# audexdev/Lossless-Audio-Codec

Hardware: AMD Instinct MI355X
Metric: encode Msamples/s at 1/2/4/8 MI355X; byte-identical .lac vs CPU ref (higher is better)
Workload: dtype int64

## Files before the change

### lossless-audio-codec_amd/csrc/analyze_core.h

```cpp
#pragma once
#include <type_traits>

#include "lacx_types.h"
#include "x87.h"

namespace lacx {

template <int CH_, int T_>
struct Geo {
    static constexpr int CH = CH_;
    static constexpr int T = T_;
    static constexpr int MAXN = CH_ * T_;
    static constexpr int LV = (CH_ == 16) ? 5 : ((CH_ == 8) ? 4 : 3);
    static constexpr int TPG = 64 / CH_;
    static constexpr int NG = MAXN / 64;
    static constexpr int W256 = 256 / CH_;
    static constexpr int W96 = 96 / CH_;
    static constexpr int MAXP = (MAXN >= 8192) ? 8 : ((MAXN >= 4096) ? 7 : ((MAXN >= 2048) ? 6 : ((MAXN >= 1024) ? 5 : ((MAXN >= 512) ? 4 : 3))));
    static constexpr int NSEG = (2 << MAXP) - 2;
    static_assert(32 % CH_ == 0, "chunk must divide the 96/256 windows");
    static_assert(MAXN % 64 == 0, "whole groups");
};

template <class G>
LACX_HD int sw(int j) {
    return (j % G::CH) * G::T + (j / G::CH);
}

enum : int { PCM_PLANAR_I32 = 0, PCM_INTERLEAVED_I16 = 1, PCM_INTERLEAVED_I24 = 2 };

struct SlotSrc {
    const int32_t* a;
    const int32_t* b;
    int kind;
    int layout = PCM_PLANAR_I32;
    int channels = 2;
};

LACX_HD int32_t sext24(uint32_t v) { return (int32_t)(v << 8) >> 8; }
LACX_HD int32_t slot_combine(int kind, int32_t l, int32_t r);

LACX_HD int32_t slot_fetch(const SlotSrc& s, int64_t idx) {
    int32_t l, r = 0;
    if (s.layout == PCM_PLANAR_I32) {
        if (s.kind == CH_L) return s.a[idx];
        if (s.kind == CH_R) return s.b[idx];
        l = s.a[idx];
        r = s.b[idx];
    } else if (s.layout == PCM_INTERLEAVED_I16) {
        if (s.channels == 2) {
            const uint32_t w = reinterpret_cast<const uint32_t*>(s.a)[idx];
            l = (int32_t)(int16_t)(w & 0xFFFFu);
            r = (int32_t)(int16_t)(w >> 16);
        } else {
            l = reinterpret_cast<const int16_t*>(s.a)[idx];
        }
    } else {
        const uint8_t* p = reinterpret_cast<const uint8_t*>(s.a) + idx * 3 * s.channels;
        l = sext24((uint32_t)p[0] | ((uint32_t)p[1] << 8) | ((uint32_t)p[2] << 16));
        if (s.channels == 2) r = sext24((uint32_t)p[3] | ((uint32_t)p[4] << 8) | ((uint32_t)p[5] << 16));
    }
    return slot_combine(s.kind, l, r);
}

LACX_HD uint32_t zigzag32(int32_t r) { return ((uint32_t)r << 1) ^ (uint32_t)(r >> 31); }

LACX_HD int opaque_i32(int v) {
#if defined(__HIP_DEVICE_COMPILE__)
    asm volatile("" : "+v"(v));
#endif
    return v;
}

LACX_HD int ctz32(uint32_t v) {
    return __builtin_ctz(v);
}

LACX_HD int clz32(uint32_t v) {
#if defined(__HIP_DEVICE_COMPILE__)
    return __clz((int)v);
#else
    return v ? __builtin_clz(v) : 32;
#endif
}

LACX_HD uint32_t kmean(uint64_t S, uint32_t c) {
    const uint64_t X = S + (c >> 1);
    const uint64_t Y = X - c;
    const int g = clz64((uint64_t)c) - clz64(Y);
    const uint32_t k = (uint32_t)g + ((Y >> (g & 63)) >= c ? 1u : 0u);
    return (X < 2ull * c) ? 0u : k;
}
LACX_HD uint32_t kmean32(uint32_t S, uint32_t c) {
    const uint32_t X = S + (c >> 1);
    const uint32_t Y = X - c;
    const int g = clz32(c) - clz32(Y);
    const uint32_t k = (uint32_t)g + ((Y >> (g & 31)) >= c ? 1u : 0u);
    return (X < 2u * c) ? 0u : k;
}

constexpr uint64_t kNarrowLimit = (1ull << 32) - (1ull << 20);

template <bool NARROW>
LACX_HD uint32_t kmean_t(uint64_t S, uint32_t c) {
    return NARROW ? kmean32((uint32_t)S, c) : kmean(S, c);
}

LACX_HD uint64_t rice_cost(uint32_t u, uint32_t k) {
    return (uint64_t)((k >= 31u) ? 0u : (u >> k)) + 1u + k;
}

LACX_HD uint32_t flag01(bool b) {
    uint32_t v = b ? 1u : 0u;
#if defined(__HIP_DEVICE_COMPILE__)
    asm volatile("" : "+v"(v));
#endif
    return v;
}

template <bool NARROW, bool STEADY = false>
LACX_HD uint32_t biased_k(uint32_t km, uint64_t P, uint64_t W, uint32_t d, uint32_t c) {
    const uint32_t L = NARROW ? ((((uint32_t)P - (uint32_t)W) + 128u) >> 8) : (uint32_t)(((P - W) + 128u) >> 8);
    const uint32_t U = (3u * L + 3u) >> 2;
    const uint32_t D = L + (L + 3u) / 3u + 1u;
    const uint64_t X = NARROW ? (uint64_t)((uint32_t)P + (c >> 1)) : P + (c >> 1);
    const uint64_t Uc = (uint64_t)U * c, Dc = (uint64_t)D * c;
    uint32_t act = flag01(X >= (uint64_t)c);
    if (!STEADY) act &= flag01(c > 256u);
    const int32_t drift = (int32_t)(act & flag01(X < Uc)) - (int32_t)(act & flag01(X >= Dc));
    const uint32_t large = d & 0xFFFFu, zero = d >> 16;
    uint32_t big = flag01(large >= 72u), sml = flag01(zero >= 77u);
    if (!STEADY) {
        const uint32_t m = flag01(c >= 96u);
        big &= m;
        sml &= m;
    }
    sml &= big ^ 1u;
    int32_t bias = drift + (int32_t)big - (int32_t)sml;
    bias = bias < -1 ? -1 : (bias > 1 ? 1 : bias);
    int bk = (int)km + bias;
    bk = bk < 0 ? 0 : (bk > 31 ? 31 : bk);
    return (uint32_t)bk;
}

struct SegInfo {
    uint64_t sbits;
    uint8_t ak;
    uint8_t sk;
    uint8_t pad[6];
};

template <class G>
struct PartMem {
    uint32_t grp[15][G::NG + 1];
    SegInfo seginfo[G::NSEG];
    unsigned long long segacc[G::NSEG][3];
    uint32_t segrun[G::NSEG];
    uint8_t choice[G::NSEG];
    unsigned long long pbits[G::MAXP + 1];
    uint32_t qcount;
    uint32_t wqcount[16];
    uint16_t queue[G::T * G::MAXP];
};

constexpr int kEmitTileWords = 12288;
template <class G>
struct EmitOut {
    uint32_t obits[kEmitTileWords];
    uint8_t kin[G::MAXN];
};
struct NoEmitOut {};

template <class G>
struct Smem {
    uint32_t u[G::MAXN + 4];
    union XP {
        int32_t x[G::MAXN];
        PartMem<G> part;
        typename std::conditional<G::T == 1024, EmitOut<G>, NoEmitOut>::type o;
    } xp;
    uint64_t tabP[G::T + 1];
    int32_t tabNZ[G::T + 1];
    uint32_t tabF[G::T + 1];
    uint16_t tabZM[G::T];
    uint16_t tabLM[G::T];
    uint16_t tabUZ[G::T + 2];
    uint16_t bqueue[G::T];
    uint32_t bqcount;
    uint32_t planeTot[2][32];
    uint32_t planeTot256[2][32];
    unsigned long long acc[2][4];
    uint32_t lbacc[11][3];
    uint32_t has4[2];
    uint64_t wtotP[16];
    int32_t wtotZ[16];
    uint32_t wtotF[16];
    uint64_t best_bits, best_rice, best_zr, best_bin, best_static;
    uint32_t best_k0, best_sk, best_hasrun;
    int32_t best_cand;
    int32_t next_cand;
    uint64_t cand_key[11];
    uint32_t cur_k0;
    LpcSet lpc;
    ChannelPlan plan;
    int32_t tabNX[G::T + 1];
    int32_t wx[16];
    uint8_t part_mode_k[kMaxParts];
    uint32_t ptype, order, p, parts, cand, header_bits, payload_bytes;
    uint32_t err;
    uint32_t plan_any_zr;
    uint32_t tmpl_state, tmpl_pad[3];
};

template <class G>
struct Thread {
    int tid;
    int a;
    uint32_t n;
    int cnt;
    uint32_t cs[G::LV];
    unsigned long long crice, cbin, czr;
    uint32_t chasrun;
    uint32_t has4;
    uint32_t umin;
    uint32_t zmask;
};

template <class G>
LACX_HD void thread_init(Thread<G>& th, uint32_t n, int tid) {
    th.tid = tid;
    th.a = tid * G::CH;
    th.n = n;
    const int rem = (int)n - th.a;
    th.cnt = rem < 0 ? 0 : (rem > G::CH ? G::CH : rem);
}

LACX_HD int32_t slot_combine(int kind, int32_t l, int32_t r) {
    if (kind == CH_L) return l;
    if (kind == CH_R) return r;
    if (kind == CH_M) return (int32_t)((uint32_t)l + (uint32_t)r) >> 1;
    return (int32_t)((uint32_t)l - (uint32_t)r);
}

struct alignas(16) Vec16 {
    uint32_t w[4];
};

template <int NV>
LACX_HD void load_vec16(const void* p, uint32_t* w ) {
    const Vec16* q = static_cast<const Vec16*>(p);
#pragma unroll
    for (int k = 0; k < NV; ++k) {
        const Vec16 t = q[k];
        w[4 * k] = t.w[0];
        w[4 * k + 1] = t.w[1];
        w[4 * k + 2] = t.w[2];
        w[4 * k + 3] = t.w[3];
    }
}

LACX_HD uint32_t bytes3(uint32_t lo, uint32_t hi, int sh) {
    const uint32_t x = sh == 0 ? lo : sh == 1 ? (lo >> 8) : sh == 2 ? ((lo >> 16) | (hi << 16)) : ((lo >> 24) | (hi << 8));
    return x & 0xFFFFFFu;
}

LACX_HD bool aligned16(const void* p) { return (reinterpret_cast<uintptr_t>(p) & 15u) == 0; }

template <int CH>
LACX_HD bool span_ok(const SlotSrc& s, int64_t first) {
    if (s.layout == PCM_PLANAR_I32) {
        const bool needa = s.kind != CH_R, needb = s.kind != CH_L;
        return CH % 4 == 0 && (!needa || aligned16(s.a + first)) && (!needb || aligned16(s.b + first));
    }
    const uint8_t* base = reinterpret_cast<const uint8_t*>(s.a);
    if (s.layout == PCM_INTERLEAVED_I16)
        return s.channels == 2 ? (CH % 4 == 0 && aligned16(base + first * 4)) : (CH % 8 == 0 && aligned16(base + first * 2));
    return CH % 16 == 0 && aligned16(base + first * (s.channels == 2 ? 6 : 3));
}

template <int CH>
LACX_HD void stage_span(const SlotSrc& s, int64_t first, int32_t* v) {
    if (s.layout == PCM_PLANAR_I32) {
        constexpr int NV = CH / 4 > 0 ? CH / 4 : 1;
        const bool needa = s.kind != CH_R, needb = s.kind != CH_L;
        uint32_t la[4 * NV] = {}, lb[4 * NV] = {};
        if (needa) load_vec16<NV>(s.a + first, la);
        if (needb) load_vec16<NV>(s.b + first, lb);
#pragma unroll
        for (int i = 0; i < CH; ++i) v[i] = slot_combine(s.kind, (int32_t)la[i], (int32_t)lb[i]);
        return;
    }
    if (s.layout == PCM_INTERLEAVED_I16) {
        if (s.channels == 2) {
            constexpr int NV = CH / 4 > 0 ? CH / 4 : 1;
            uint32_t w[4 * NV];
            load_vec16<NV>(reinterpret_cast<const uint8_t*>(s.a) + first * 4, w);
#pragma unroll
            for (int i = 0; i < CH; ++i)
                v[i] = slot_combine(s.kind, (int32_t)(int16_t)(w[i] & 0xFFFFu), (int32_t)(int16_t)(w[i] >> 16));
            return;
        }
        constexpr int NV = CH / 8 > 0 ? CH / 8 : 1;
        uint32_t w[4 * NV];
        load_vec16<NV>(reinterpret_cast<const uint8_t*>(s.a) + first * 2, w);
#pragma unroll
        for (int i = 0; i < CH; ++i) v[i] = (int32_t)(int16_t)((w[(i / 2) % (4 * NV)] >> (16 * (i & 1))) & 0xFFFFu);
        return;
    }
    if (s.channels == 2) {
        constexpr int ND = CH * 6 / 4 >= 4 ? CH * 6 / 4 : 4;
        uint32_t w[ND];
        load_vec16<ND / 4>(reinterpret_cast<const uint8_t*>(s.a) + first * 6, w);
#pragma unroll
        for (int i = 0; i < CH; ++i) {
            const int ol = (i * 6) % (ND * 4), orr = (i * 6 + 3) % (ND * 4);
            v[i] = slot_combine(s.kind, sext24(bytes3(w[ol / 4], w[(ol / 4 + 1 < ND) ? ol / 4 + 1 : ol / 4], ol & 3)),
                                sext24(bytes3(w[orr / 4], w[(orr / 4 + 1 < ND) ? orr / 4 + 1 : orr / 4], orr & 3)));
        }
        return;
    }
    constexpr int ND = CH * 3 / 4 >= 4 ? CH * 3 / 4 : 4;
    uint32_t w[ND];
    load_vec16<ND / 4>(reinterpret_cast<const uint8_t*>(s.a) + first * 3, w);
#pragma unroll
    for (int i = 0; i < CH; ++i) {
        const int o = (i * 3) % (ND * 4);
        v[i] = sext24(bytes3(w[o / 4], w[(o / 4 + 1 < ND) ? o / 4 + 1 : o / 4], o & 3));
    }
}

LACX_HD bool wave_all(bool pred) {
#if defined(__HIP_DEVICE_COMPILE__)
    return __all(pred) != 0;
#else
    return pred;
#endif
}

template <int CH>
LACX_HD void load_chunk(const SlotSrc& src, int64_t first, int cnt, int64_t last, int32_t* v) {
    if (wave_all(cnt == CH && span_ok<CH>(src, first))) {
        stage_span<CH>(src, first, v);
        return;
    }
#pragma unroll
    for (int i = 0; i < CH; ++i) {
        const int64_t idx = first + i;
        v[i] = slot_fetch(src, idx < last ? idx : last);
    }
}

template <class G, class M>
LACX_HD uint32_t stage_samples(const Thread<G>& th, M& sh, const SlotSrc& src, int64_t start) {
    int32_t v[G::CH];
    load_chunk<G::CH>(src, start + th.a, th.cnt, start + (int64_t)th.n - 1, v);
    int32_t* col = &sh.xp.x[th.tid];
    uint32_t any = 0;
#pragma unroll
    for (int i = 0; i < G::CH; ++i) {
        const int32_t x = (i < th.cnt) ? v[i] : 0;
        col[i * G::T] = x;
        any |= (uint32_t)x;
    }
    return any;
}

template <int W>
LACX_HD void sliced_add(const uint32_t* a, const uint32_t* b, uint32_t* out ) {
    uint32_t carry = 0;
#pragma unroll
    for (int l = 0; l < W; ++l) {
        const uint32_t x = a[l] ^ b[l];
        out[l] = x ^ carry;
        carry = (a[l] & b[l]) | (x & carry);
    }
    out[W] = carry;
}

template <class G>
LACX_HD void plane_counts(const uint32_t* u, uint32_t* cs) {
    if (G::CH == 16) {
        uint32_t l1[8][2], l2[4][3], l3[2][4], l4[5];
#pragma unroll
        for (int i = 0; i < 8; ++i) sliced_add<1>(&u[2 * i], &u[2 * i + 1], l1[i]);
#pragma unroll
        for (int i = 0; i < 4; ++i) sliced_add<2>(l1[2 * i], l1[2 * i + 1], l2[i]);
#pragma unroll
        for (int i = 0; i < 2; ++i) sliced_add<3>(l2[2 * i], l2[2 * i + 1], l3[i]);
        sliced_add<4>(l3[0], l3[1], l4);
#pragma unroll
        for (int l = 0; l < G::LV; ++l) cs[l] = l4[l];
    } else {
        uint32_t l1[2][2], l2[3];
        sliced_add<1>(&u[0], &u[1], l1[0]);
        sliced_add<1>(&u[2], &u[3], l1[1]);
        sliced_add<2>(l1[0], l1[1], l2);
#pragma unroll
        for (int l = 0; l < G::LV; ++l) cs[l] = l2[l];
    }
}

template <class G, class M>
LACX_HD void phase_r_residual(Thread<G>& th, const M& sh, int cand, uint32_t* u ) {
    int32_t xh[G::CH + 12];
#pragma unroll
    for (int i = 0; i < G::CH + 12; ++i) {
        const int d = i - 12;
        const int co = (d >= 0) ? d / G::CH : -((-d + G::CH - 1) / G::CH);
        const int el = d - co * G::CH;
        const int tt = th.tid + co;
        const int32_t* col = &sh.xp.x[tt < 0 ? 0 : tt];
        xh[i] = (tt >= 0) ? col[el * G::T] : 0;
    }
    const int32_t* x = xh + 12;
    if (cand <= 4) {
        auto fixed = [&](auto order_tag) {
            constexpr int K = decltype(order_tag)::value;
#pragma unroll
            for (int i = 0; i < G::CH; ++i) {
                const uint32_t x0 = (uint32_t)x[i], x1 = (uint32_t)x[i - 1], x2 = (uint32_t)x[i - 2],
                               x3 = (uint32_t)x[i - 3], x4 = (uint32_t)x[i - 4];
                uint32_t r = x0;
                if (K == 1) r = x0 - x1;
                if (K == 2) r = x0 - 2u * x1 + x2;
                if (K == 3) r = x0 - 3u * x1 + 3u * x2 - x3;
                if (K == 4) r = x0 - 4u * x1 + 6u * x2 - 4u * x3 + x4;
                if (K > 0 && th.a + i < K) r = x0;
                u[i] = (i < th.cnt) ? zigzag32((int32_t)r) : 0u;
            }
        };
        if (cand == 0) fixed(std::integral_constant<int, 0>{});
        else if (cand == 1) fixed(std::integral_constant<int, 1>{});
        else if (cand == 2) fixed(std::integral_constant<int, 2>{});
        else if (cand == 3) fixed(std::integral_constant<int, 3>{});
        else fixed(std::integral_constant<int, 4>{});
    } else if (cand == 5) {
#pragma unroll
        for (int i = 0; i < G::CH; ++i) {
            const int j = th.a + i;
            const int64_t pred = (3LL * (int64_t)x[i - 1] - (int64_t)x[i - 2]) >> 2;
            const int32_t r = (j >= 2) ? (int32_t)((int64_t)x[i] - pred) : x[i];
            u[i] = (i < th.cnt) ? zigzag32(r) : 0u;
        }
    } else {
        const int ci = cand - 6;
        const int ord = sh.lpc.used[ci];
        auto lpc = [&](auto taps_tag) {
            constexpr int TAPS = decltype(taps_tag)::value;
            int32_t c[TAPS + 1];
#pragma unroll
            for (int t = 1; t <= TAPS; ++t) c[t] = (t <= ord) ? (int32_t)sh.lpc.coef[ci][t] : 0;
#pragma unroll
            for (int i = 0; i < G::CH; ++i) {
                int64_t acc = 0;
#pragma unroll
                for (int t = 1; t <= TAPS; ++t) acc += (int64_t)c[t] * (int64_t)x[i - t];
                const int32_t r = (int32_t)((int64_t)x[i] - (acc >> 15));
                u[i] = (i < th.cnt) ? zigzag32(r) : 0u;
            }
        };
        if (ord <= 4) lpc(std::integral_constant<int, 4>{});
        else if (ord <= 6) lpc(std::integral_constant<int, 6>{});
        else if (ord <= 8) lpc(std::integral_constant<int, 8>{});
        else if (ord <= 10) lpc(std::integral_constant<int, 10>{});
        else lpc(std::integral_constant<int, 12>{});
    }
}

template <class G, class M>
LACX_HD void phase_r_store(Thread<G>& th, M& sh, const uint32_t* u) {
    uint64_t s = 0;
    int32_t lastnz = -1;
#pragma unroll
    for (int i = 0; i < G::CH; ++i) {
        s += u[i];
        if (u[i] != 0) lastnz = th.a + i;
        sh.u[i * G::T + th.tid] = u[i];
    }
    sh.tabP[th.tid] = s;
    sh.tabNZ[th.tid] = lastnz;
    plane_counts<G>(u, th.cs);
}

template <class G, class M>
LACX_HD void phase_r(Thread<G>& th, M& sh, int cand) {
    uint32_t u[G::CH];
    phase_r_residual(th, sh, cand, u);
    phase_r_store(th, sh, u);
}

LACX_HD uint32_t lead_m(int32_t r) {
#if defined(__HIP_DEVICE_COMPILE__)
    uint32_t f;
    asm("v_ffbh_i32 %0, %1" : "=v"(f) : "v"(r));
    return f < 32u ? f : 32u;
#else
    const uint32_t v = (uint32_t)(r ^ (r >> 31));
    return v ? (uint32_t)__builtin_clz(v) : 32u;
#endif
}

struct BoundPartials {
    uint32_t msum;
#if defined(__HIP_DEVICE_COMPILE__)
    uint32_t code;
#else
    uint32_t nz;
    uint32_t n4;
    uint32_t ends;
    uint32_t zprev;
#endif
};

LACX_HD void bound_init(BoundPartials& b) {
#if defined(__HIP_DEVICE_COMPILE__)
    b.msum = b.code = 0;
#else
    b.msum = b.nz = b.n4 = b.ends = b.zprev = 0;
#endif
}

LACX_HD void bound_add(BoundPartials& b, int32_t r) {
    b.msum += lead_m(r);
#if defined(__HIP_DEVICE_COMPILE__)
    const uint32_t v = (uint32_t)r;
    b.code = (b.code << 2) + (v < 3u ? v : 3u);
#else
    const uint32_t z = r == 0 ? 1u : 0u;
    b.nz += z;
    b.ends += (b.zprev && !z) ? 1u : 0u;
    b.zprev = z;
    b.n4 += r == 2 ? 1u : 0u;
#endif
}

template <int CH>
LACX_HD uint32_t bound_counts(const BoundPartials& b) {
    static_assert(CH <= 16, "two bits per position in one word");
#if defined(__HIP_DEVICE_COMPILE__)
    constexpr uint32_t kLow = CH == 16 ? 0x55555555u : ((1u << (2 * (CH & 15))) - 1u) & 0x55555555u;
    const uint32_t lo = b.code & kLow, hi = (b.code >> 1) & kLow;
    const uint32_t zero = ~(lo | hi) & kLow;
    const uint32_t four = hi & ~lo;
    const uint32_t ends = zero & ~(zero << 2) & ~1u;
    return (uint32_t)__builtin_popcount(zero) | ((uint32_t)__builtin_popcount(four) << 11) |
           ((uint32_t)__builtin_popcount(ends) << 22);
#else
    return b.nz | (b.n4 << 11) | (b.ends << 22);
#endif
}

template <class G, class M>
LACX_HD void pass1_window(const Thread<G>& th, const M& sh, int32_t* xh ) {
#pragma unroll
    for (int i = 0; i < G::CH + 12; ++i) {
        const int d = i - 12;
        const int co = (d >= 0) ? d / G::CH : -((-d + G::CH - 1) / G::CH);
        const int el = d - co * G::CH;
        const int tt = th.tid + co;
        const int32_t* col = &sh.xp.x[tt < 0 ? 0 : tt];
        xh[i] = (tt >= 0) ? col[el * G::T] : 0;
    }
}

template <class G, bool FULL, class M>
LACX_HD void pass1_bounds_fixed(const Thread<G>& th, const M& sh, BoundPartials* out ) {
    int32_t xh[G::CH + 12];
    pass1_window(th, sh, xh);
    const int32_t* x = xh + 12;
    const bool first = th.a == 0;
    auto live = [&](int i, int32_t r) { return FULL ? r : ((i < th.cnt) ? r : 0); };
    {
        BoundPartials b[6];
#pragma unroll
        for (int c = 0; c < 6; ++c) bound_init(b[c]);
        const uint32_t e1 = (uint32_t)x[-1] - (uint32_t)x[-2], e1b = (uint32_t)x[-2] - (uint32_t)x[-3],
                       e1c = (uint32_t)x[-3] - (uint32_t)x[-4];
        const uint32_t e2 = e1 - e1b, e2b = e1b - e1c;
        uint32_t p1 = e1, p2 = e2, p3 = e2 - e2b;
#pragma unroll
        for (int i = 0; i < G::CH; ++i) {
            const uint32_t x0 = (uint32_t)x[i];
            const uint32_t d1 = x0 - (uint32_t)x[i - 1], d2 = d1 - p1, d3 = d2 - p2, d4 = d3 - p3;
            p1 = d1;
            p2 = d2;
            p3 = d3;
            const int32_t fir = (int32_t)(x0 - (uint32_t)((3 * x[i - 1] - x[i - 2]) >> 2));
            const bool w1 = first && i < 1, w2 = first && i < 2, w3 = first && i < 3, w4 = first && i < 4;
            bound_add(b[0], live(i, (int32_t)x0));
            bound_add(b[1], live(i, (int32_t)(w1 ? x0 : d1)));
            bound_add(b[2], live(i, (int32_t)(w2 ? x0 : d2)));
            bound_add(b[3], live(i, (int32_t)(w3 ? x0 : d3)));
            bound_add(b[4], live(i, (int32_t)(w4 ? x0 : d4)));
            bound_add(b[5], live(i, w2 ? (int32_t)x0 : fir));
        }
#pragma unroll
        for (int c = 0; c < 6; ++c) out[c] = b[c];
    }
}

template <class G, bool FULL, class M>
LACX_HD void pass1_bounds_lpc(const Thread<G>& th, const M& sh, bool lpc_off, BoundPartials* out ) {
    int32_t xh[G::CH + 12];
    pass1_window(th, sh, xh);
    const int32_t* x = xh + 12;
    auto live = [&](int i, int32_t r) { return FULL ? r : ((i < th.cnt) ? r : 0); };
    for (int ci = 0; ci < 5; ++ci) {
        BoundPartials b;
        bound_init(b);
        const int ord = lpc_off ? 0 : (int)sh.lpc.used[ci];
        auto lpc = [&](auto taps_tag) {
            constexpr int TAPS = decltype(taps_tag)::value;
            int32_t c[TAPS + 1];
#pragma unroll
            for (int t = 1; t <= TAPS; ++t) c[t] = (t <= ord) ? (int32_t)sh.lpc.coef[ci][t] : 0;
#pragma unroll
            for (int i = 0; i < G::CH; ++i) {
                int64_t acc = 0;
#pragma unroll
                for (int t = 1; t <= TAPS; ++t) acc += (int64_t)c[t] * (int64_t)x[i - t];
                const int32_t r = (int32_t)((uint32_t)x[i] - (uint32_t)((uint64_t)acc >> 15));
                bound_add(b, live(i, r));
                }
        };
        if (ord == 0) {
        } else if (ord <= 4) lpc(std::integral_constant<int, 4>{});
        else if (ord <= 6) lpc(std::integral_constant<int, 6>{});
        else if (ord <= 8) lpc(std::integral_constant<int, 8>{});
        else if (ord <= 10) lpc(std::integral_constant<int, 10>{});
        else lpc(std::integral_constant<int, 12>{});
#pragma unroll
        for (int c = 0; c < 5; ++c) {
            if (c == ci) out[c] = b;
        }
    }
}

template <class G, bool FULL, class M>
LACX_HD void pass1_bounds(const Thread<G>& th, const M& sh, bool lpc_off, BoundPartials* out ) {
    pass1_bounds_fixed<G, FULL>(th, sh, out);
    pass1_bounds_lpc<G, FULL>(th, sh, lpc_off, out + 6);
}

LACX_HD void planes_to_ksums(const uint32_t* C, uint64_t* A, int kmax) {
    uint64_t acc = 0;
#pragma unroll
    for (int b = 29; b >= 0; --b) {
        acc = (acc << 1) + C[b];
        if (b <= 15) A[b] = (b <= kmax) ? acc : 0;
    }
}

LACX_HD uint32_t pick_initial_k(const uint64_t* A, uint32_t m) {
    uint32_t best_k = 0;
    uint64_t best = ~0ull;
#pragma unroll
    for (uint32_t k = 0; k <= 12; ++k) {
        const uint64_t c = A[k] + (uint64_t)m * (1u + k);
        if (c < best) {
            best = c;
            best_k = k;
        }
    }
    return best_k;
}

LACX_HD uint32_t pick_static_k(const uint64_t* A, uint32_t m, uint64_t* bits) {
    uint32_t best_k = 0;
    uint64_t best = ~0ull;
#pragma unroll
    for (uint32_t k = 0; k <= 15; ++k) {
        const uint64_t c = A[k] + (uint64_t)m * (1u + k);
        if (c < best) {
            best = c;
            best_k = k;
        }
    }
    *bits = best;
    return best_k;
}

template <class G, bool NARROW, class M>
LACX_HD void phase_a(Thread<G>& th, M& sh) {
    uint64_t P = sh.tabP[th.tid];
    uint32_t cnt = 0;
    uint32_t c = (uint32_t)th.a;
    uint32_t zm = 0;
    uint32_t mn = 0xFFFFFFFFu;
    uint32_t fzm = 0;
    uint32_t flm = 0;
    for (int i = 0; i < th.cnt; ++i) {
        const uint32_t u = sh.u[i * G::T + th.tid];
        mn = u < mn ? u : mn;
        P += u;
        ++c;
        const uint32_t km = kmean_t<NARROW>(P, c);
        const uint32_t q = u >> km;
        const uint32_t fl = q > 3u, fz = q == 0u;
        cnt += fl + (fz << 16);
        zm |= (u == 0u ? 1u : 0u) << i;
        fzm |= fz << i;
        flm |= fl << i;
    }
    sh.tabF[th.tid] = cnt;
    sh.tabZM[th.tid] = (uint16_t)fzm;
    sh.tabLM[th.tid] = (uint16_t)flm;
    if constexpr (requires { sh.tabUZ[0]; }) sh.tabUZ[th.tid] = (uint16_t)zm;
    th.umin = mn;
    th.zmask = zm;
    const uint32_t lead = (uint32_t)ctz32(~zm);
    const int32_t before = th.a - 1 - sh.tabNZ[th.tid];
    th.has4 = (th.cnt > 0 && ((zm & (zm >> 1) & (zm >> 2) & (zm >> 3)) != 0u || (uint32_t)before + lead >= 4u)) ? 1u : 0u;
}

template <class G, class M>
LACX_HD uint32_t peek_u(const M& sh, uint32_t j, uint32_t limit) {
    const uint32_t idx = (j % (uint32_t)G::CH) * (uint32_t)G::T + (j / (uint32_t)G::CH);
    const uint32_t v = sh.u[idx] & 0x3FFFFFFFu;
    return (j < limit) ? v : 1u;
}

template <class G>
LACX_HD uint32_t window_flags(const uint32_t* tabF, int t) {
    uint32_t d = 0;
#pragma unroll
    for (int k = 1; k <= G::W96; ++k) d += (t >= k) ? tabF[t - k] : 0u;
    return d;
}

struct ChunkCosts {
    unsigned long long rice, bin, zr;
    uint32_t hasrun;
};

template <class G, bool NARROW, bool ZR = true, int TRIPS = 0, bool STEADY = false>
LACX_HD ChunkCosts phase_b_span(const Smem<G>& sh, uint32_t n, int t, int i0, int i1, uint32_t k0) {
    const int a = t * G::CH;
    uint64_t P = sh.tabP[t];
    uint64_t W = (STEADY || t >= G::W256) ? sh.tabP[t - (STEADY || t >= G::W256 ? G::W256 : 0)] : 0;
    uint32_t D = window_flags<G>(sh.tabF, t);
    const uint32_t m256 = (STEADY || t >= G::W256) ? 0xFFFFFFFFu : 0u;
    const int t256 = (STEADY || t >= G::W256) ? t - G::W256 : t;
    const int t96 = (STEADY || t >= G::W96) ? t - G::W96 : t;
    const uint32_t fin = (uint32_t)sh.tabLM[t] | ((uint32_t)sh.tabZM[t] << 16);
    const uint32_t fout = (STEADY || t >= G::W96) ? ((uint32_t)sh.tabLM[t96] | ((uint32_t)sh.tabZM[t96] << 16)) : 0u;
    uint32_t c = (uint32_t)a;
    int32_t f = a - 1 - sh.tabNZ[t];
    for (int j = 0; j < i0; ++j) {
        const uint32_t u = sh.u[j * G::T + t];
        P += u;
        ++c;
        W += sh.u[j * G::T + t256] & m256;
        D += (fin >> j) & 0x00010001u;
        D -= (fout >> j) & 0x00010001u;
        f = (f + 1) & (int32_t)(0u - flag01(u == 0u));
    }
    uint32_t kin = k0;
    if (STEADY || (c > 0u && i1 > i0)) kin = biased_k<NARROW, STEADY>(kmean_t<NARROW>(P, c), P, W, D, c);
    using Acc = typename std::conditional<NARROW, uint32_t, unsigned long long>::type;
    Acc rice = 0, bin = 0, zr = 0;
    uint32_t hasrun = 0;
    const int ifirst = i0 & (G::CH - 1);
    uint32_t w0 = sh.u[ifirst * G::T + t];
    uint32_t n1 = 1, n2 = 1, n3 = 1;
    if (ZR) {
        n1 = peek_u<G>(sh, (uint32_t)(a + i0) + 1u, n);
        n2 = peek_u<G>(sh, (uint32_t)(a + i0) + 2u, n);
        n3 = peek_u<G>(sh, (uint32_t)(a + i0) + 3u, n);
    }
    uint32_t tap256 = sh.u[ifirst * G::T + t256];
    const int last = TRIPS > 0 ? i0 + TRIPS : i1;
#pragma nounroll
    for (int i = i0; i < last; ++i) {
        const uint32_t cur256 = tap256;
        const int inext = (i + 1) & (G::CH - 1);
        const uint32_t wnext = sh.u[inext * G::T + t];
        tap256 = sh.u[inext * G::T + t256];
        const uint32_t u = w0;
        const uint32_t rc = (u >> kin) + 1u + kin;
        rice += rc;
        bin += 2u + ((u <= 4u) ? (u < 1u ? u : 1u) : rc);
        if (ZR) {
            const uint32_t z = flag01(u == 0u);
            f = (f + 1) & (int32_t)(0u - z);
            const uint32_t ahead = (n1 != 0) ? 0u : ((n2 != 0) ? 1u : ((n3 != 0) ? 2u : 3u));
            const uint32_t in4 = z & flag01((uint32_t)f + ahead >= 4u);
            const uint32_t esc = 1u << ((kin + 3u) < 24u ? (kin + 3u) : 24u);
            const uint32_t plain = 2u + ((u > esc) ? 32u : rc);
            const uint32_t token = 5u + (((uint32_t)(f - 4)) >> 2);
            const uint32_t runend = in4 & flag01(n1 != 0);
            zr += (plain & (in4 - 1u)) | (token & (0u - runend));
            hasrun |= runend;
        }
        P += u;
        ++c;
        W += cur256 & m256;
        D += (fin >> i) & 0x00010001u;
        D -= (fout >> i) & 0x00010001u;
        kin = biased_k<NARROW, STEADY>(kmean_t<NARROW>(P, c), P, W, D, c);
        w0 = wnext;
        if (ZR) {
            n1 = n2;
            n2 = n3;
            n3 = peek_u<G>(sh, (uint32_t)(a + i) + 4u, n);
        }
    }
    ChunkCosts out;
    out.rice = rice;
    out.bin = bin;
    out.zr = zr;
    out.hasrun = hasrun;
    return out;
}

template <class G, bool NARROW, bool ZR = true, bool FULL = false, bool STEADY = false>
LACX_HD void phase_b(Thread<G>& th, const Smem<G>& sh, uint32_t k0) {
    const ChunkCosts cc = phase_b_span<G, NARROW, ZR, FULL ? G::CH : 0, STEADY>(sh, th.n, th.tid, 0, th.cnt, k0);
    th.crice = cc.rice;
    th.cbin = cc.bin;
    th.czr = cc.zr;
    th.chasrun = cc.hasrun;
}

template <class G>
LACX_HD void phase_b_dispatch(Thread<G>& th, const Smem<G>& sh, uint32_t k0, bool narrow, bool zr, bool full, bool steady) {
    auto go = [&](auto narrow_t, auto zr_t) {
        constexpr bool N = decltype(narrow_t)::value, Z = decltype(zr_t)::value;
        if (full) {
            if (steady) phase_b<G, N, Z, true, true>(th, sh, k0); else phase_b<G, N, Z, true, false>(th, sh, k0);
        } else {
            if (steady) phase_b<G, N, Z, false, true>(th, sh, k0); else phase_b<G, N, Z, false, false>(th, sh, k0);
        }
    };
    if (narrow) {
        if (zr) go(std::true_type{}, std::true_type{}); else go(std::true_type{}, std::false_type{});
    } else {
        if (zr) go(std::false_type{}, std::true_type{}); else go(std::false_type{}, std::false_type{});
    }
}
template <class G>
LACX_HD void phase_b_dispatch(Thread<G>& th, const Smem<G>& sh, uint32_t k0, bool narrow, bool zr, bool full) {
    phase_b_dispatch<G>(th, sh, k0, narrow, zr, full, G::T > 64 && th.tid >= 64 && 64 * G::CH >= 256);
}

#ifndef LACX_QUEUED_STEADY
#define LACX_QUEUED_STEADY 1
#endif
template <class G>
LACX_HD void phase_b_queued(Thread<G>& th, const Smem<G>& sh, int t, uint32_t k0, bool narrow, bool zr, bool full) {
    Thread<G> c;
    thread_init(c, th.n, t);
    phase_b_dispatch<G>(c, sh, k0, narrow, zr, full, LACX_QUEUED_STEADY != 0);
    th.crice += c.crice;
    th.cbin += c.cbin;
    th.czr += c.czr;
    th.chasrun |= c.chasrun;
}

LACX_HD uint32_t census_code(uint32_t u);
LACX_HD uint32_t census_shift_sum(uint32_t cen, uint32_t K);

struct RunShape {
    uint32_t nin4, tokens, hasrun, first_in4;
};
template <int CH>
LACX_HD RunShape run_shape(uint32_t E, int32_t f) {
    RunShape r{0u, 0u, 0u, 0u};
#pragma unroll
    for (int i = 0; i < CH; ++i) {
        const uint32_t z = (E >> i) & 1u;
        f = (f + 1) & (int32_t)(0u - z);
        const uint32_t after = E >> (i + 1);
        const uint32_t ahead = (after & 1u) == 0u ? 0u : ((after & 2u) == 0u ? 1u : ((after & 4u) == 0u ? 2u : 3u));
        const uint32_t in4 = z & flag01((uint32_t)f + ahead >= 4u);
        const uint32_t runend = in4 & ((after & 1u) ^ 1u);
        r.nin4 += in4;
        r.tokens += (5u + (((uint32_t)(f - 4)) >> 2)) & (0u - runend);
        r.hasrun |= runend;
        if (i == 0) r.first_in4 = in4;
    }
    return r;
}

template <class G, bool NARROW, bool ZR>
LACX_HD bool phase_b_quick(Thread<G>& th, const Smem<G>& sh) {
    if constexpr (G::T <= 64 || 64 * G::CH <= 256) {
        return false;
    } else {
        const int t = th.tid;
        if (t < 64 || th.cnt != G::CH) return false;
        using Sum = typename std::conditional<NARROW, uint32_t, uint64_t>::type;
        const Sum P0 = (Sum)sh.tabP[t], P1 = (Sum)sh.tabP[t + 1];
        const Sum W0 = (Sum)sh.tabP[t - G::W256], W1 = (Sum)sh.tabP[t - G::W256 + 1];
        const uint32_t c0 = (uint32_t)th.a, c1 = c0 + (uint32_t)G::CH;
        const uint32_t km = kmean_t<NARROW>(P0, c1);
        uint32_t ok = flag01(km == kmean_t<NARROW>(P1, c0));
        const uint32_t Llo = (uint32_t)(((P0 - W1) + 128u) >> 8), Lhi = (uint32_t)(((P1 - W0) + 128u) >> 8);
        const uint32_t Ulo = (3u * Llo + 3u) >> 2, Uhi = (3u * Lhi + 3u) >> 2;
        const uint32_t Dlo = Llo + (Llo + 3u) / 3u + 1u, Dhi = Lhi + (Lhi + 3u) / 3u + 1u;
        const uint64_t Xlo = NARROW ? (uint64_t)((uint32_t)P0 + (c0 >> 1)) : (uint64_t)P0 + (c0 >> 1);
        const uint64_t Xhi = NARROW ? (uint64_t)((uint32_t)P1 + (c1 >> 1)) : (uint64_t)P1 + (c1 >> 1);
        const uint32_t act_never = flag01(Xhi < (uint64_t)c0), act_always = flag01(Xlo >= (uint64_t)c1);
        const uint32_t up_always = flag01(Xhi < (uint64_t)Ulo * c0), up_never = flag01(Xlo >= (uint64_t)Uhi * c1);
        const uint32_t dn_always = flag01(Xlo >= (uint64_t)Dhi * c1), dn_never = flag01(Xhi < (uint64_t)Dlo * c0);
        ok &= act_never | (act_always & (up_always | up_never) & (dn_always | dn_never));
        const int32_t drift = (int32_t)((act_never ^ 1u) & up_always) - (int32_t)((act_never ^ 1u) & dn_always);
        const uint32_t d0 = window_flags<G>(sh.tabF, t), din = sh.tabF[t], dout = sh.tabF[t - G::W96];
        const int32_t l0 = (int32_t)(d0 & 0xFFFFu), z0 = (int32_t)(d0 >> 16);
        const uint32_t big_always = flag01(l0 - (int32_t)(dout & 0xFFFFu) >= 72), big_never = flag01(l0 + (int32_t)(din & 0xFFFFu) < 72);
        uint32_t sml_always, sml_never;
        {
            const uint32_t zin = sh.tabZM[t], zout = sh.tabZM[t - G::W96];
            int32_t z = z0, zmin = z0, zmax = z0;
#pragma unroll
            for (int i = 0; i + 1 < G::CH; ++i) {
                z += (int32_t)((zin >> i) & 1u) - (int32_t)((zout >> i) & 1u);
                zmin = z < zmin ? z : zmin;
                zmax = z > zmax ? z : zmax;
            }
            sml_always = flag01(zmin >= 77);
            sml_never = flag01(zmax < 77);
        }
        ok &= big_always | (big_never & (sml_always | sml_never));
        int32_t bias = drift + (int32_t)big_always - (int32_t)((big_always ^ 1u) & sml_always);
        bias = bias < -1 ? -1 : (bias > 1 ? 1 : bias);
        int bk = (int)km + bias;
        bk = bk < 0 ? 0 : (bk > 31 ? 31 : bk);
        const uint32_t k = (uint32_t)bk;
        uint32_t any = 0;
        Sum ksum = 0;
#pragma unroll
        for (int l = 0; l < G::LV; ++l) {
            any |= th.cs[l];
            ksum += (Sum)(th.cs[l] >> k) << l;
        }
        if (ZR) ok &= flag01((any >> ((k + 3u) < 24u ? (k + 3u) : 24u)) == 0u);
        if (ok == 0u) return false;
        const Sum rice = ksum + (uint32_t)G::CH * (1u + k);
        uint32_t n14 = 0, nbig = (uint32_t)G::CH, small_shifted = 0;
        if (th.umin <= 4u) {
            uint32_t cen = 0;
#pragma unroll
            for (int i = 0; i < G::CH; ++i) cen += census_code(sh.u[i * G::T + t] & 0x3FFFFFFFu);
            n14 = ((cen >> 5) & 31u) + ((cen >> 10) & 31u) + ((cen >> 15) & 31u) + ((cen >> 20) & 31u);
            nbig = (cen >> 25) & 31u;
            small_shifted = census_shift_sum(cen, k);
        }
        th.crice = rice;
        th.cbin = (Sum)(2u * (uint32_t)G::CH + n14 + nbig * (1u + k)) + (ksum - small_shifted);
        RunShape rs{0u, 0u, 0u, 0u};
        if (ZR && th.zmask != 0u)
            rs = run_shape<G::CH>(th.zmask | (((uint32_t)sh.tabUZ[t + 1] & 7u) << G::CH), th.a - 1 - sh.tabNZ[t]);
        const uint32_t nin4 = rs.nin4, tokens = rs.tokens, hasrun = rs.hasrun;
        th.czr = ksum + (Sum)(((uint32_t)G::CH - nin4) * (3u + k) + tokens);
        th.chasrun = hasrun;
        return true;
    }
}

template <class G>
LACX_HD bool phase_b_quick_dispatch(Thread<G>& th, const Smem<G>& sh, bool narrow, bool zr) {
    if (narrow) return zr ? phase_b_quick<G, true, true>(th, sh) : phase_b_quick<G, true, false>(th, sh);
    return zr ? phase_b_quick<G, false, true>(th, sh) : phase_b_quick<G, false, false>(th, sh);
}

LACX_HD uint64_t candidate_lower_bound(uint32_t g_sum, uint32_t aux_sum, uint32_t ends, uint32_t n, int zero_run) {
    const uint32_t nzero = aux_sum & 0xFFFFu, n4 = aux_sum >> 16;
    const uint64_t lb_rice = g_sum;
    const uint64_t lb_bin = (uint64_t)g_sum - n4;
    uint64_t lb = lb_rice < lb_bin ? lb_rice : lb_bin;
    if (zero_run) {
        uint64_t zeros = 0;
        if (nzero != 0) {
            const uint32_t runs = ends > 1u ? ends : 1u;
            const uint64_t shorts = 3ull * nzero, one_long = 3ull * (runs - 1u) + 4u + ((nzero - runs + 1u) >> 2);
            zeros = shorts < one_long ? shorts : one_long;
        }
        const uint64_t lb_zr = (uint64_t)g_sum - nzero + 2ull * (n - nzero) + zeros;
        if (lb_zr < lb) lb = lb_zr;
    }
    return lb;
}

LACX_HD int candidate_at(int i) { return (int)((0x405316789A2ull >> (4 * i)) & 15ull); }

LACX_HD bool candidate_pruned(uint64_t lb, int cand, uint64_t best_bits, int best_cand) {
    return best_cand >= 0 && (lb > best_bits || (lb == best_bits && cand > best_cand));
}

template <class G>
LACX_HD void score_candidate(Smem<G>& sh, int cand, uint32_t n, int zero_run, uint32_t k0,
                             const uint32_t* planeTot, const unsigned long long* acc) {
    uint64_t A[16];
    planes_to_ksums(planeTot, A, 15);
    uint64_t sbits;
    const uint32_t sk = pick_static_k(A, n, &sbits);
    const uint64_t rice = acc[0], bin = acc[1];
    const uint32_t hasrun = acc[3] != 0;
    const uint64_t zr = (zero_run && hasrun) ? acc[2] : rice;
    uint64_t a = rice < sbits ? rice : sbits;
    uint64_t b = zr < bin ? zr : bin;
    const uint64_t best = a < b ? a : b;
    if (sh.best_cand < 0 || best < sh.best_bits || (best == sh.best_bits && cand < sh.best_cand)) {
        sh.best_cand = cand;
        sh.best_bits = best;
        sh.best_rice = rice;
        sh.best_zr = zr;
        sh.best_bin = bin;
        sh.best_static = sbits;
        sh.best_k0 = k0;
        sh.best_sk = sk;
        sh.best_hasrun = hasrun;
    }
}

LACX_HD uint32_t initial_k_from_planes(const uint32_t* planes256, uint32_t n) {
    uint64_t A[16];
    planes_to_ksums(planes256, A, 12);
    return pick_initial_k(A, n < 256u ? n : 256u);
}

LACX_HD int max_partition_order(uint32_t n) {
    int mp = 0;
    for (int p = 1; p <= kMaxPartitionOrder; ++p) {
        if ((n >> p) < (uint32_t)kMinPartition) break;
        mp = p;
    }
    return mp;
}

template <class G>
LACX_HD void packed_planes(const Thread<G>& th, uint32_t* words ) {
#pragma unroll
    for (int w = 0; w < 15; ++w) {
        uint32_t v = 0;
#pragma unroll
        for (int l = 0; l < G::LV; ++l) {
            v += (((th.cs[l] >> w) & 1u) << l) + (((th.cs[l] >> (w + 15)) & 1u) << (16 + l));
        }
        words[w] = v;
    }
}

template <class G>
LACX_HD void range_ksums(const Smem<G>& sh, uint32_t s, uint32_t e, uint64_t* A) {
#pragma unroll
    for (int k = 0; k < 16; ++k) A[k] = 0;
    const uint32_t gs = (s + 63u) >> 6, ge = e >> 6;
    uint32_t e0 = e, s1 = e;
    if (gs < ge) {
        uint32_t C[30];
#pragma unroll
        for (int w = 0; w < 15; ++w) {
            const uint32_t d = sh.xp.part.grp[w][ge] - sh.xp.part.grp[w][gs];
            C[w] = d & 0xFFFFu;
            C[w + 15] = d >> 16;
        }
        planes_to_ksums(C, A, 15);
        e0 = gs << 6;
        s1 = ge << 6;
    }
    for (uint32_t j = s; j < e0; ++j) {
        const uint32_t u = sh.u[sw<G>((int)j)];
#pragma unroll
        for (int k = 0; k < 16; ++k) A[k] += u >> k;
    }
    for (uint32_t j = s1; j < e; ++j) {
        const uint32_t u = sh.u[sw<G>((int)j)];
#pragma unroll
        for (int k = 0; k < 16; ++k) A[k] += u >> k;
    }
}

LACX_HD void seg_bounds(uint32_t n, int p, uint32_t part, uint32_t* s, uint32_t* e) {
    const uint32_t base = n >> p, parts = 1u << p;
    *s = part * base;
    *e = (part + 1u == parts) ? n : (*s + base);
}

template <class G>
LACX_HD void seg_static_eval(Smem<G>& sh, uint32_t n, int p, uint32_t part) {
    uint32_t s, e;
    seg_bounds(n, p, part, &s, &e);
    const uint32_t len = e - s;
    uint64_t A[16];
    range_ksums(sh, s, e, A);
    SegInfo si;
    si.sk = (uint8_t)pick_static_k(A, len, &si.sbits);
    const uint32_t m = len < 256u ? len : 256u;
    if (m != len) range_ksums(sh, s, s + m, A);
    si.ak = (uint8_t)pick_initial_k(A, m);
    for (int i = 0; i < 6; ++i) si.pad[i] = 0;
    sh.xp.part.seginfo[(2u << (p - 1)) - 2u + part] = si;
}

template <class G, bool NARROW, bool ZR = true, class Flush>
LACX_HD void partition_pass(const Thread<G>& th, const Smem<G>& sh, int p, Flush&& flush) {
    if (th.cnt <= 0) return;
    const uint32_t n = th.n;
    const uint32_t base = n >> p, parts = 1u << p;
    uint32_t part = (uint32_t)th.a / base;
    if (part >= parts) part = parts - 1u;
    uint32_t s = part * base;
    uint32_t e = (part + 1u == parts) ? n : s + base;
    const uint32_t segbase = (2u << (p - 1)) - 2u;
    uint64_t P = sh.tabP[th.tid];
    uint64_t Pseg;
    {
        const uint32_t cs = s / G::CH;
        Pseg = sh.tabP[cs];
        for (uint32_t j = cs * G::CH; j < s; ++j) Pseg += sh.u[sw<G>((int)j)];
    }
    int32_t lastnz = sh.tabNZ[th.tid];
    if (lastnz < (int32_t)s - 1) lastnz = (int32_t)s - 1;
    int32_t f = th.a - 1 - lastnz;
    unsigned long long rice = 0, bin = 0, zr = 0;
    uint32_t hasrun = 0;
    uint32_t u = sh.u[th.tid];
    uint32_t x1 = peek_u<G>(sh, (uint32_t)th.a + 1u, n), x2 = peek_u<G>(sh, (uint32_t)th.a + 2u, n),
             x3 = peek_u<G>(sh, (uint32_t)th.a + 3u, n);
    for (int i = 0; i < th.cnt; ++i) {
        const uint32_t j = (uint32_t)(th.a + i);
        if (j == e) {
            flush(segbase + part, rice, bin, zr, hasrun);
            rice = bin = zr = 0;
            hasrun = 0;
            ++part;
            s = e;
            e = (part + 1u == parts) ? n : s + base;
            Pseg = P;
            f = 0;
        }
        const uint32_t kin = (j == s) ? (uint32_t)sh.xp.part.seginfo[segbase + part].ak
                                      : kmean_t<NARROW>(P - Pseg, j - s);
        const uint32_t rc = ((kin >= 31u) ? 0u : (u >> kin)) + 1u + kin;
        rice += rc;
        bin += (u == 0) ? 2u : ((u <= 4u) ? 3u : 2u + rc);
        if (ZR) {
            const bool z = (u == 0);
            f = z ? f + 1 : 0;
            const uint32_t n1 = (j + 1u < e) ? x1 : 1u;
            const uint32_t n2 = (j + 2u < e) ? x2 : 1u;
            const uint32_t n3 = (j + 3u < e) ? x3 : 1u;
            const int ahead = (n1 != 0) ? 0 : ((n2 != 0) ? 1 : ((n3 != 0) ? 2 : 3));
            const bool in4 = z && (f + ahead >= 4);
            if (!in4) {
                const uint32_t esc = 1u << ((kin + 3u) < 24u ? (kin + 3u) : 24u);
                zr += 2u + ((u > esc) ? 32u : rc);
            } else if (n1 != 0) {
                zr += 2u + (((uint32_t)(f - 4)) >> 2) + 3u;
                hasrun = 1;
            }
        }
        P += u;
        u = x1;
        x1 = x2;
        x2 = x3;
        x3 = peek_u<G>(sh, (uint32_t)(th.a + i) + 4u, n);
    }
    flush(segbase + part, rice, bin, zr, hasrun);
}


template <class G>
LACX_HD bool partitions_chunk_aligned(uint32_t n, int max_p) {
    return max_p > 0 && (n % ((uint32_t)G::CH << max_p)) == 0u;
}

template <class G, bool ZR = true, class Flush>
LACX_HD void partition_fused(const Thread<G>& th, const Smem<G>& sh, int max_p, Flush&& flush) {
    const bool live = th.cnt > 0;
    const uint32_t n = th.n;
    const int t = th.tid;
    const uint32_t a = (uint32_t)th.a;
    const uint32_t Pa = (uint32_t)sh.tabP[t];
    uint32_t s[G::MAXP], rem[G::MAXP], Pseg[G::MAXP], ak[G::MAXP], sidx[G::MAXP];
    uint32_t rice[G::MAXP], bin[G::MAXP], zr[G::MAXP];
    uint32_t hasrun = 0;
#pragma unroll
    for (int q = 0; q < G::MAXP; ++q) {
        const int p = q + 1;
        rice[q] = bin[q] = zr[q] = 0;
        s[q] = rem[q] = Pseg[q] = ak[q] = sidx[q] = 0;
        if (p <= max_p) {
            const uint32_t base = n >> p;
            const uint32_t part = !live ? 0u : ((n & (n - 1u)) == 0u ? a >> (31 - clz32(n) - p) : a / base);
            s[q] = part * base;
            rem[q] = s[q] + base - a;
            Pseg[q] = (uint32_t)sh.tabP[s[q] / (uint32_t)G::CH];
            sidx[q] = (2u << (p - 1)) - 2u + part;
            ak[q] = sh.xp.part.seginfo[sidx[q]].ak;
        }
    }
    uint32_t dup = 0;
    if (!ZR) {
#pragma unroll
        for (int q = 1; q < G::MAXP; ++q)
            if (q < max_p && wave_all(s[q] == s[q - 1] && ak[q] == ak[q - 1])) dup |= 1u << q;
    }
    int32_t fg = (int32_t)a - 1 - sh.tabNZ[t];
    uint32_t P = Pa;
    uint32_t u = sh.u[t];
    uint32_t x1 = peek_u<G>(sh, a + 1u, n), x2 = peek_u<G>(sh, a + 2u, n), x3 = peek_u<G>(sh, a + 3u, n);
    auto sample = [&](int i, auto first_tag) {
        constexpr bool FIRST = decltype(first_tag)::value;
        const uint32_t j = a + (uint32_t)i;
        const bool z = (u == 0);
        fg = z ? fg + 1 : 0;
        const uint32_t ahead_g = (x1 != 0) ? 0u : ((x2 != 0) ? 1u : ((x3 != 0) ? 2u : 3u));
        const uint32_t small = (u == 0) ? 2u : 3u;
        const bool is_small = u <= 4u;
#pragma unroll
        for (int q = 0; q < G::MAXP; ++q) {
            if (q < max_p && !((dup >> q) & 1u)) {
                const uint32_t cbefore = j - s[q];
                uint32_t kin = kmean32(P - Pseg[q], FIRST ? (cbefore ? cbefore : 1u) : cbefore);
                if (FIRST) kin = (cbefore == 0) ? ak[q] : kin;
                const uint32_t rc = (u >> kin) + 1u + kin;
                rice[q] += rc;
                bin[q] += is_small ? small : 2u + rc;
                if (ZR) {
                    const uint32_t left = rem[q] - 1u - (uint32_t)i;
                    const uint32_t fp = ((uint32_t)fg < cbefore + 1u) ? (uint32_t)fg : cbefore + 1u;
                    const uint32_t ahead = ahead_g < left ? ahead_g : left;
                    const bool in4 = z & (fp + ahead >= 4u);
                    const bool runend = in4 & (ahead == 0u);
                    const uint32_t esc = 1u << ((kin + 3u) < 24u ? (kin + 3u) : 24u);
                    const uint32_t plain = 2u + ((u > esc) ? 32u : rc);
                    const uint32_t token = 5u + ((fp - 4u) >> 2);
                    zr[q] += in4 ? (runend ? token : 0u) : plain;
                    hasrun |= runend ? (1u << q) : 0u;
                }
            }
        }
        P += u;
        u = x1;
        x1 = x2;
        x2 = x3;
        x3 = peek_u<G>(sh, j + 4u, n);
    };
    if (live) {
        sample(0, std::true_type{});
        for (int i = 1; i < th.cnt; ++i) sample(i, std::false_type{});
    }
#pragma unroll
    for (int q = 1; q < G::MAXP; ++q) {
        if ((dup >> q) & 1u) {
            rice[q] = rice[q - 1];
            bin[q] = bin[q - 1];
        }
    }
#pragma unroll
    for (int q = 0; q < G::MAXP; ++q) {
        if (q < max_p) flush(q, sidx[q], rice[q], bin[q], zr[q], (hasrun >> q) & 1u);
    }
}

LACX_HD uint32_t census_code(uint32_t u) { return 1u << (5u * (u < 5u ? u : 5u)); }

template <class G>
LACX_HD uint32_t small_census(const Thread<G>& th, const Smem<G>& sh, uint32_t* u_first, uint32_t* zmask) {
    uint32_t cen = 0, zm = 0;
#pragma unroll
    for (int i = 0; i < G::CH; ++i) {
        const uint32_t u = sh.u[i * G::T + th.tid];
        if (i == 0) *u_first = u;
        cen += census_code(u);
        zm |= flag01(u == 0u) << i;
    }
    *zmask = zm;
    return cen;
}

LACX_HD uint32_t census_shift_sum(uint32_t cen, uint32_t K) {
    const uint32_t n1 = (cen >> 5) & 31u, n2 = (cen >> 10) & 31u, n3 = (cen >> 15) & 31u, n4 = (cen >> 20) & 31u;
    const uint32_t s0 = n1 + 2u * n2 + 3u * n3 + 4u * n4, s1 = n2 + n3 + 2u * n4, s2 = n4;
    return K == 0u ? s0 : (K == 1u ? s1 : (K == 2u ? s2 : 0u));
}

template <class G, class Flush, class Enqueue>
LACX_HD void partition_quick(const Thread<G>& th, const Smem<G>& sh, int max_p, Flush&& flush, Enqueue&& enqueue) {
    const bool live = th.cnt > 0;
    const uint32_t n = th.n;
    const int t = th.tid;
    const uint32_t a = (uint32_t)th.a;
    const uint32_t Pa = (uint32_t)sh.tabP[t];
    const uint32_t csum = (uint32_t)sh.tabP[t + 1] - Pa;
    uint32_t u_first;
    uint32_t zmask_unused;
    const uint32_t cen = small_census(th, sh, &u_first, &zmask_unused);
    const uint32_t u_last = sh.u[(G::CH - 1) * G::T + t];
    const uint32_t code_first = census_code(u_first);
    const bool n_pow2 = (n & (n - 1u)) == 0u;
    const int log2n = 31 - clz32(n);
    for (int q = 0; q < max_p; ++q) {
        const int p = q + 1;
        const uint32_t base = n >> p;
        const uint32_t part = !live ? 0u : (n_pow2 ? a >> (log2n - p) : a / base);
        const uint32_t s = part * base;
        const uint32_t sidx = (2u << (p - 1)) - 2u + part;
        const uint32_t Sa = Pa - (uint32_t)sh.tabP[s / (uint32_t)G::CH];
        const uint32_t ca = a - s;
        const bool head = ca == 0u;
        const uint32_t klo = kmean32(head ? u_first : Sa, ca + (uint32_t)G::CH - 1u);
        const uint32_t khi = kmean32(Sa + csum - u_last, head ? 1u : ca);
        const bool ambiguous = live && klo != khi;
        enqueue((uint32_t)t | ((uint32_t)q << 12), ambiguous);
        const bool quick = live && !ambiguous;
        const uint32_t K = klo;
        uint32_t shifted = 0;
#pragma unroll
        for (int l = 0; l < G::LV; ++l) shifted += (th.cs[l] >> K) << l;
        const uint32_t k_a = (uint32_t)sh.xp.part.seginfo[sidx].ak;
        const uint32_t rc_a = (u_first >> k_a) + 1u + k_a;
        const uint32_t ncon = (uint32_t)G::CH - (head ? 1u : 0u);
        const uint32_t cen_con = cen - (head ? code_first : 0u);
        if (head) shifted -= u_first >> K;
        const uint32_t rice = shifted + ncon * (1u + K) + (head ? rc_a : 0u);
        const uint32_t n14 = ((cen_con >> 5) & 31u) + ((cen_con >> 10) & 31u) + ((cen_con >> 15) & 31u) + ((cen_con >> 20) & 31u);
        const uint32_t nbig = (cen_con >> 25) & 31u;
        const uint32_t bin_a = 2u + (u_first <= 4u ? (u_first < 1u ? u_first : 1u) : rc_a);
        const uint32_t bin = 2u * ncon + n14 + (shifted - census_shift_sum(cen_con, K)) + nbig * (1u + K) + (head ? bin_a : 0u);
        flush(q, sidx, quick ? rice : 0u, quick ? bin : 0u, 0u, 0u);
    }
}

template <class G>
struct QuickPrep {
    uint32_t Pa, u_first, cen, code_first;
    uint32_t E;
    int32_t f0;
    RunShape rs;
    uint32_t amb;
    uint32_t Kpack[(G::MAXP + 3) / 4];
};

constexpr uint32_t kQuickMaxPairs = 256;

template <class G>
LACX_HD void partition_quick_prepare(const Thread<G>& th, const Smem<G>& sh, int max_p, QuickPrep<G>& qp) {
    const bool live = th.cnt > 0;
    const uint32_t n = th.n;
    const int t = th.tid;
    const uint32_t a = (uint32_t)th.a;
    qp.Pa = (uint32_t)sh.tabP[t];
    const uint32_t csum = (uint32_t)sh.tabP[t + 1] - qp.Pa;
    uint32_t zmask;
    qp.cen = small_census(th, sh, &qp.u_first, &zmask);
    const uint32_t u_last = sh.u[(G::CH - 1) * G::T + t];
    qp.code_first = census_code(qp.u_first);
    qp.E = zmask | (flag01(peek_u<G>(sh, a + (uint32_t)G::CH, n) == 0u) << G::CH) |
           (flag01(peek_u<G>(sh, a + (uint32_t)G::CH + 1u, n) == 0u) << (G::CH + 1)) |
           (flag01(peek_u<G>(sh, a + (uint32_t)G::CH + 2u, n) == 0u) << (G::CH + 2));
    qp.f0 = (int32_t)a - 1 - sh.tabNZ[t];
    qp.rs = run_shape<G::CH>(qp.E, qp.f0);
    uint32_t any = 0;
#pragma unroll
    for (int l = 0; l < G::LV; ++l) any |= th.cs[l];
    const bool n_pow2 = (n & (n - 1u)) == 0u;
    const int log2n = 31 - clz32(n);
    qp.amb = 0;
#pragma unroll
    for (int w = 0; w < (G::MAXP + 3) / 4; ++w) qp.Kpack[w] = 0;
#pragma unroll
    for (int q = 0; q < G::MAXP; ++q) {
        if (q >= max_p) continue;
        const int p = q + 1;
        const uint32_t base = n >> p;
        const uint32_t part = !live ? 0u : (n_pow2 ? a >> (log2n - p) : a / base);
        const uint32_t s = part * base;
        const uint32_t Sa = qp.Pa - (uint32_t)sh.tabP[s / (uint32_t)G::CH];
        const uint32_t ca = a - s;
        const bool head = ca == 0u;
        const uint32_t klo = kmean32(head ? qp.u_first : Sa, ca + (uint32_t)G::CH - 1u);
        const uint32_t khi = kmean32(Sa + csum - u_last, head ? 1u : ca);
        const bool cut_front = (qp.E & 1u) != 0u && (uint32_t)qp.f0 > ca;
        const bool cut_back = ca + (uint32_t)G::CH == base && ((qp.E >> (G::CH - 1)) & 3u) == 3u;
        const bool escape = (any >> ((klo + 3u) < 24u ? (klo + 3u) : 24u)) != 0u;
        const bool ambiguous = klo != khi || (cut_front && head) || cut_back || escape;
        qp.Kpack[q >> 2] |= klo << (8 * (q & 3));
        qp.amb |= (live && ambiguous) ? (1u << q) : 0u;
    }
}

template <class G, class Flush, class Enqueue>
LACX_HD void partition_quick_costs(const Thread<G>& th, const Smem<G>& sh, int max_p, const QuickPrep<G>& qp, Flush&& flush,
                                   Enqueue&& enqueue) {
    const bool live = th.cnt > 0;
    const uint32_t n = th.n;
    const int t = th.tid;
    const uint32_t a = (uint32_t)th.a;
    const bool n_pow2 = (n & (n - 1u)) == 0u;
    const int log2n = 31 - clz32(n);
    const uint32_t open_run = (uint32_t)ctz32(~qp.E);
#pragma unroll
    for (int q = 0; q < G::MAXP; ++q) {
        if (q >= max_p) continue;
        const int p = q + 1;
        const uint32_t base = n >> p;
        const uint32_t part = !live ? 0u : (n_pow2 ? a >> (log2n - p) : a / base);
        const uint32_t sidx = (2u << (p - 1)) - 2u + part;
        const uint32_t ca = a - part * base;
        const bool head = ca == 0u;
        const bool ambiguous = ((qp.amb >> q) & 1u) != 0u;
        enqueue((uint32_t)t | ((uint32_t)q << 12), ambiguous);
        const bool quick = live && !ambiguous;
        const uint32_t K = (qp.Kpack[q >> 2] >> (8 * (q & 3))) & 0xFFu;
        uint32_t shifted = 0;
#pragma unroll
        for (int l = 0; l < G::LV; ++l) shifted += (th.cs[l] >> K) << l;
        const uint32_t k_a = (uint32_t)sh.xp.part.seginfo[sidx].ak;
        const uint32_t rc_a = (qp.u_first >> k_a) + 1u + k_a;
        const uint32_t ncon = (uint32_t)G::CH - (head ? 1u : 0u);
        const uint32_t cen_con = qp.cen - (head ? qp.code_first : 0u);
        if (head) shifted -= qp.u_first >> K;
        const uint32_t rice = shifted + ncon * (1u + K) + (head ? rc_a : 0u);
        const uint32_t n14 = ((cen_con >> 5) & 31u) + ((cen_con >> 10) & 31u) + ((cen_con >> 15) & 31u) + ((cen_con >> 20) & 31u);
        const uint32_t nbig = (cen_con >> 25) & 31u;
        const uint32_t bin_a = 2u + (qp.u_first <= 4u ? (qp.u_first < 1u ? qp.u_first : 1u) : rc_a);
        const uint32_t bin = 2u * ncon + n14 + (shifted - census_shift_sum(cen_con, K)) + nbig * (1u + K) + (head ? bin_a : 0u);
        const bool head_plain = head && qp.rs.first_in4 == 0u;
        const uint32_t esc_a = 1u << ((k_a + 3u) < 24u ? (k_a + 3u) : 24u);
        const uint32_t plain_a = 2u + (qp.u_first > esc_a ? 32u : rc_a);
        const uint32_t nplain = (uint32_t)G::CH - qp.rs.nin4 - (head_plain ? 1u : 0u);
        uint32_t tokens = qp.rs.tokens;
        if ((qp.E & 1u) != 0u && (uint32_t)qp.f0 > ca && !head && open_run <= (uint32_t)G::CH)
            tokens = tokens + ((ca + open_run - 4u) >> 2) - (((uint32_t)qp.f0 + open_run - 4u) >> 2);
        const uint32_t zr = shifted + nplain * (3u + K) + (head_plain ? plain_a : 0u) + tokens;
        flush(q, sidx, quick ? rice : 0u, quick ? bin : 0u, quick ? zr : 0u, quick ? qp.rs.hasrun : 0u);
    }
}

template <class G, bool ZR = false, class Flush>
LACX_HD void partition_slow_entry(const Smem<G>& sh, uint32_t n, uint32_t entry, Flush&& flush) {
    const uint32_t t = entry & 0xFFFu;
    const int p = (int)(entry >> 12) + 1;
    const uint32_t a = t * (uint32_t)G::CH;
    const uint32_t base = n >> p;
    const uint32_t part = (n & (n - 1u)) == 0u ? a >> (31 - clz32(n) - p) : a / base;
    const uint32_t s = part * base;
    const uint32_t sidx = (2u << (p - 1)) - 2u + part;
    uint32_t S = (uint32_t)sh.tabP[t] - (uint32_t)sh.tabP[s / (uint32_t)G::CH];
    uint32_t c = a - s;
    uint32_t k = c == 0u ? (uint32_t)sh.xp.part.seginfo[sidx].ak : kmean32(S, c ? c : 1u);
    uint32_t rice = 0, bin = 0, zr = 0, hasrun = 0;
    uint32_t u = sh.u[t];
    int32_t fg = (int32_t)a - 1 - sh.tabNZ[t];
    uint32_t x1 = 1, x2 = 1, x3 = 1;
    if (ZR) {
        x1 = peek_u<G>(sh, a + 1u, n);
        x2 = peek_u<G>(sh, a + 2u, n);
        x3 = peek_u<G>(sh, a + 3u, n);
    }
#pragma unroll
    for (int i = 0; i < G::CH; ++i) {
        const uint32_t unext = ZR ? x1 : sh.u[((i + 1) & (G::CH - 1)) * G::T + t];
        const uint32_t rc = (u >> k) + 1u + k;
        rice += rc;
        bin += 2u + (u <= 4u ? (u < 1u ? u : 1u) : rc);
        if (ZR) {
            const uint32_t z = flag01(u == 0u);
            fg = (fg + 1) & (int32_t)(0u - z);
            const uint32_t ahead_g = (x1 != 0) ? 0u : ((x2 != 0) ? 1u : ((x3 != 0) ? 2u : 3u));
            const uint32_t left = base - 1u - c;
            const uint32_t fp = ((uint32_t)fg < c + 1u) ? (uint32_t)fg : c + 1u;
            const uint32_t ahead = ahead_g < left ? ahead_g : left;
            const uint32_t in4 = z & flag01(fp + ahead >= 4u);
            const uint32_t runend = in4 & flag01(ahead == 0u);
            const uint32_t esc = 1u << ((k + 3u) < 24u ? (k + 3u) : 24u);
            const uint32_t plain = 2u + ((u > esc) ? 32u : rc);
            const uint32_t token = 5u + ((fp - 4u) >> 2);
            zr += (plain & (in4 - 1u)) | (token & (0u - runend));
            hasrun |= runend;
            x1 = x2;
            x2 = x3;
            x3 = peek_u<G>(sh, a + (uint32_t)i + 4u, n);
        }
        S += u;
        ++c;
        k = kmean32(S, c);
        u = unext;
    }
    flush(sidx, rice, bin, zr, hasrun);
}

template <class G>
LACX_HD uint64_t seg_choose(Smem<G>& sh, uint32_t idx, int zero_run) {
    PartMem<G>& pm = sh.xp.part;
    const SegInfo si = pm.seginfo[idx];
    const uint64_t normal = pm.segacc[idx][0], bin = pm.segacc[idx][1];
    const bool allow_zr = zero_run && pm.segrun[idx] != 0;
    const uint64_t zr = allow_zr ? pm.segacc[idx][2] : normal;
    uint32_t mode = 0, k = si.ak;
    uint64_t bits = normal;
    if (allow_zr && zr < bits) {
        mode = 1;
        bits = zr;
    }
    if (bin < bits) {
        mode = 2;
        bits = bin;
    }
    if (si.sbits < bits || si.sbits <= bits + bits / 20u) {
        mode = 3;
        k = si.sk;
        bits = si.sbits;
    }
    pm.choice[idx] = (uint8_t)((mode << 5) | k);
    return bits;
}

template <class G>
LACX_HD void finalize_plan(Smem<G>& sh, uint32_t n, int zero_run, int max_p, ChannelPlan* out) {
    const int cand = sh.best_cand;
    uint8_t ptype, order;
    if (cand <= 4) {
        ptype = 0;
        order = (uint8_t)cand;
    } else if (cand == 5) {
        ptype = 1;
        order = 2;
    } else {
        ptype = 2;
        order = sh.lpc.used[cand - 6];
    }
    out->valid = 1;
    out->predictor_type = ptype;
    out->order = order;
    for (int i = 0; i < 12; ++i) out->coef[i] = (cand >= 6) ? sh.lpc.coef[cand - 6][i + 1] : (int16_t)0;
    const bool allow_zr = zero_run && sh.best_hasrun;
    uint32_t mode = 0, k = sh.best_k0;
    uint64_t bits = sh.best_rice;
    if (allow_zr && sh.best_zr <= bits) {
        bits = sh.best_zr;
        mode = 1;
    }
    if (sh.best_bin < bits) {
        bits = sh.best_bin;
        mode = 2;
    }
    if (sh.best_static < bits) {
        bits = sh.best_static;
        mode = 3;
        k = sh.best_sk;
    }
    uint64_t best_total = bits + 8u + 7u;
    best_total += (8u - (best_total & 7u)) & 7u;
    int best_p = 0;
    for (int p = 1; p <= max_p; ++p) {
        uint64_t total = sh.xp.part.pbits[p] + 8u + 7ull * (1u << p);
        total += (8u - (total & 7u)) & 7u;
        const uint64_t margin = best_total / 20u;
        if (total < best_total || (total <= best_total + margin && best_p == 0)) {
            best_total = total;
            best_p = p;
        }
    }
    out->partition_order = (uint8_t)best_p;
    out->total_bits = best_total;
    out->payload_bytes = (uint32_t)((16u + (ptype == 2 ? 16u * order : 0u) + best_total) >> 3);
    uint32_t any_zr = 0;
    if (best_p == 0) {
        out->part_mode_k[0] = (uint8_t)((mode << 5) | k);
        any_zr = mode == 1u;
    } else {
        const uint32_t parts = 1u << best_p, segbase = (2u << (best_p - 1)) - 2u;
        for (uint32_t i = 0; i < parts; ++i) {
            const uint8_t c = sh.xp.part.choice[segbase + i];
            out->part_mode_k[i] = c;
            any_zr |= (uint32_t)((c >> 5) == 1u);
        }
    }
    sh.plan_any_zr = any_zr;
}

}
```

### lossless-audio-codec_amd/csrc/device_util.h

```cpp
#pragma once
#include <hip/hip_runtime.h>

#include "analyze_core.h"
#include "kernels.h"

namespace lacx {

#ifdef LACX_STAMPS
extern __device__ unsigned long long g_stamp_acc[40];
#define STAMP(k)                                                        \
    do {                                                                \
        const unsigned long long _now = __builtin_amdgcn_s_memtime();   \
        stamp_acc[k] += _now - stamp_prev;                              \
        stamp_prev = _now;                                              \
    } while (0)
#define STAMP_PARAMS , unsigned long long* stamp_acc, unsigned long long& stamp_prev
#define STAMP_ARGS , stamp_acc, stamp_prev
#else
#define STAMP(k) do { } while (0)
#define STAMP_PARAMS
#define STAMP_ARGS
#endif
constexpr int kDppRowShr1 = 0x111, kDppRowShr2 = 0x112, kDppRowShr4 = 0x114, kDppRowShr8 = 0x118;
constexpr int kDppRowBcast15 = 0x142, kDppRowBcast31 = 0x143;

template <int CTRL, int ROW_MASK>
__device__ __forceinline__ uint32_t dpp_mov(uint32_t identity, uint32_t v) {
    return (uint32_t)__builtin_amdgcn_update_dpp((int)identity, (int)v, CTRL, ROW_MASK, 0xF, false);
}
template <int CTRL, int ROW_MASK>
__device__ __forceinline__ uint64_t dpp_mov64(uint64_t v) {
    const uint32_t lo = dpp_mov<CTRL, ROW_MASK>(0u, (uint32_t)v);
    const uint32_t hi = dpp_mov<CTRL, ROW_MASK>(0u, (uint32_t)(v >> 32));
    return ((uint64_t)hi << 32) | lo;
}

__device__ __forceinline__ uint32_t wave_scan_add_u32(uint32_t v) {
    v += dpp_mov<kDppRowShr1, 0xF>(0u, v);
    v += dpp_mov<kDppRowShr2, 0xF>(0u, v);
    v += dpp_mov<kDppRowShr4, 0xF>(0u, v);
    v += dpp_mov<kDppRowShr8, 0xF>(0u, v);
    v += dpp_mov<kDppRowBcast15, 0xA>(0u, v);
    v += dpp_mov<kDppRowBcast31, 0xC>(0u, v);
    return v;
}
__device__ __forceinline__ uint64_t wave_scan_add_u64(uint64_t v) {
    v += dpp_mov64<kDppRowShr1, 0xF>(v);
    v += dpp_mov64<kDppRowShr2, 0xF>(v);
    v += dpp_mov64<kDppRowShr4, 0xF>(v);
    v += dpp_mov64<kDppRowShr8, 0xF>(v);
    v += dpp_mov64<kDppRowBcast15, 0xA>(v);
    v += dpp_mov64<kDppRowBcast31, 0xC>(v);
    return v;
}
__device__ __forceinline__ int32_t wave_scan_max_i32(int32_t v) {
    constexpr uint32_t kMin = 0x80000000u;
    auto mx = [](int32_t a, uint32_t b) { return a > (int32_t)b ? a : (int32_t)b; };
    v = mx(v, dpp_mov<kDppRowShr1, 0xF>(kMin, (uint32_t)v));
    v = mx(v, dpp_mov<kDppRowShr2, 0xF>(kMin, (uint32_t)v));
    v = mx(v, dpp_mov<kDppRowShr4, 0xF>(kMin, (uint32_t)v));
    v = mx(v, dpp_mov<kDppRowShr8, 0xF>(kMin, (uint32_t)v));
    v = mx(v, dpp_mov<kDppRowBcast15, 0xA>(kMin, (uint32_t)v));
    v = mx(v, dpp_mov<kDppRowBcast31, 0xC>(kMin, (uint32_t)v));
    return v;
}
__device__ __forceinline__ uint32_t wave_scan_or_u32(uint32_t v) {
    v |= dpp_mov<kDppRowShr1, 0xF>(0u, v);
    v |= dpp_mov<kDppRowShr2, 0xF>(0u, v);
    v |= dpp_mov<kDppRowShr4, 0xF>(0u, v);
    v |= dpp_mov<kDppRowShr8, 0xF>(0u, v);
    v |= dpp_mov<kDppRowBcast15, 0xA>(0u, v);
    v |= dpp_mov<kDppRowBcast31, 0xC>(0u, v);
    return v;
}
__device__ __forceinline__ uint64_t wave_scan_min_u64(uint64_t v) {
    auto step = [](uint64_t a, uint32_t lo, uint32_t hi) {
        const uint64_t b = ((uint64_t)hi << 32) | lo;
        return b < a ? b : a;
    };
#define LACX_MIN_STEP(CTRL, MASK) \
    v = step(v, dpp_mov<CTRL, MASK>(0xFFFFFFFFu, (uint32_t)v), dpp_mov<CTRL, MASK>(0xFFFFFFFFu, (uint32_t)(v >> 32)))
    LACX_MIN_STEP(kDppRowShr1, 0xF);
    LACX_MIN_STEP(kDppRowShr2, 0xF);
    LACX_MIN_STEP(kDppRowShr4, 0xF);
    LACX_MIN_STEP(kDppRowShr8, 0xF);
    LACX_MIN_STEP(kDppRowBcast15, 0xA);
    LACX_MIN_STEP(kDppRowBcast31, 0xC);
#undef LACX_MIN_STEP
    return v;
}
__device__ __forceinline__ uint32_t wave_last_u32(uint32_t v) { return (uint32_t)__builtin_amdgcn_readlane((int)v, 63); }
__device__ __forceinline__ uint64_t wave_last_u64(uint64_t v) {
    return ((uint64_t)wave_last_u32((uint32_t)(v >> 32)) << 32) | wave_last_u32((uint32_t)v);
}
__device__ __forceinline__ uint64_t wave_sum_u64(uint64_t v) { return wave_last_u64(wave_scan_add_u64(v)); }
__device__ __forceinline__ uint32_t wave_sum_u32(uint32_t v) { return wave_last_u32(wave_scan_add_u32(v)); }
__device__ __forceinline__ uint32_t wave_or_u32(uint32_t v) { return wave_last_u32(wave_scan_or_u32(v)); }

template <int LOG>
__device__ __forceinline__ uint32_t seg_sum_u32(uint32_t v) {
    if (LOG >= 1) v += dpp_mov<kDppRowShr1, 0xF>(0u, v);
    if (LOG >= 2) v += dpp_mov<kDppRowShr2, 0xF>(0u, v);
    if (LOG >= 3) v += dpp_mov<kDppRowShr4, 0xF>(0u, v);
    if (LOG >= 4) v += dpp_mov<kDppRowShr8, 0xF>(0u, v);
    if (LOG >= 5) v += dpp_mov<kDppRowBcast15, 0xA>(0u, v);
    if (LOG >= 6) v += dpp_mov<kDppRowBcast31, 0xC>(0u, v);
    return v;
}
__device__ __forceinline__ uint32_t seg_sum_u32(uint32_t v, int log2_lanes) {
    switch (log2_lanes) {
        case 1: return seg_sum_u32<1>(v);
        case 2: return seg_sum_u32<2>(v);
        case 3: return seg_sum_u32<3>(v);
        case 4: return seg_sum_u32<4>(v);
        case 5: return seg_sum_u32<5>(v);
        default: return seg_sum_u32<6>(v);
    }
}

template <class G>
struct ScanRegs {
    uint64_t v, inc;
    int32_t z, zinc;
};

template <class G, class M>
__device__ __forceinline__ void scan_pz_part1(M& sh, int tid, ScanRegs<G>& r) {
    const int lane = tid & 63, wave = tid >> 6;
    r.v = sh.tabP[tid];
    r.z = sh.tabNZ[tid];
    const uint64_t inc = wave_scan_add_u64(r.v);
    const int32_t zinc = wave_scan_max_i32(r.z);
    r.inc = inc;
    r.zinc = zinc;
    if (lane == 63) {
        sh.wtotP[wave] = inc;
        sh.wtotZ[wave] = zinc;
    }
}

template <class G, class M>
__device__ __forceinline__ uint64_t scan_pz_part2(M& sh, int tid, const ScanRegs<G>& r) {
    const int lane = tid & 63, wave = tid >> 6;
    uint64_t base = 0, total = 0;
    int32_t zbase = -1;
#pragma unroll
    for (int w = 0; w < G::T / 64; ++w) {
        const uint64_t pw = sh.wtotP[w];
        const int32_t z = sh.wtotZ[w];
        total += pw;
        if (w < wave) {
            base += pw;
            zbase = z > zbase ? z : zbase;
        }
    }
    int32_t zprev = __shfl_up(r.zinc, 1, 64);
    if (lane == 0) zprev = -1;
    sh.tabP[tid] = base + r.inc - r.v;
    sh.tabNZ[tid] = zprev > zbase ? zprev : zbase;
    if (tid == G::T - 1) {
        sh.tabP[G::T] = base + r.inc;
        sh.tabNZ[G::T] = r.zinc > zbase ? r.zinc : zbase;
    }
    return total;
}

template <class G>
__device__ __forceinline__ void plane_totals_wave(const Thread<G>& th, uint32_t* planeTot, uint32_t* planeTot256,
                                                  int tid, int first_plane = 0) {
    const int lane = tid & 63, wave = tid >> 6;
    uint32_t any = 0;
#pragma unroll
    for (int l = 0; l < G::LV; ++l) any |= th.cs[l];
    const int nplanes = 32 - __clz((int)wave_or_u32(any));
    const uint64_t m256 = (G::W256 >= 64) ? ~0ull : ((1ull << (G::W256 & 63)) - 1ull);
    uint32_t mine = 0, mine256 = 0;
    const bool first256 = wave == 0;
    for (int b = first256 ? 0 : first_plane; b < nplanes; ++b) {
        uint32_t tot = 0, tot256 = 0;
#pragma unroll
        for (int l = 0; l < G::LV; ++l) {
            const uint64_t m = __ballot((th.cs[l] >> b) & 1u);
            tot += (uint32_t)__popcll(m) << l;
            if (first256) tot256 += (uint32_t)__popcll(m & m256) << l;
        }
        if (lane == b) {
            mine = tot;
            mine256 = tot256;
        }
    }
    if (lane < nplanes) {
        if (lane >= first_plane) atomicAdd(&planeTot[lane], mine);
        if (wave == 0) atomicAdd(&planeTot256[lane], mine256);
    }
}

template <class G>
__device__ __forceinline__ void ksums_wave(const Thread<G>& th, uint32_t* ksum, uint32_t* ksum256, int tid, uint32_t kmask = 0xFFFFu) {
    const int lane = tid & 63, wave = tid >> 6;
    static_assert(G::W256 == 16 || G::W256 == 64, "the first 256 samples are one DPP row or the whole wave");
#pragma unroll
    for (int k = 0; k < 16; ++k) {
        const bool wanted = ((kmask >> k) & 1u) != 0u;
        const bool head256 = wave == 0 && k <= 12;
        if (!wanted && !head256) continue;
        uint32_t v = 0;
#pragma unroll
        for (int l = 0; l < G::LV; ++l) v += (th.cs[l] >> k) << l;
        v += dpp_mov<kDppRowShr1, 0xF>(0u, v);
        v += dpp_mov<kDppRowShr2, 0xF>(0u, v);
        v += dpp_mov<kDppRowShr4, 0xF>(0u, v);
        v += dpp_mov<kDppRowShr8, 0xF>(0u, v);
        const uint32_t row = v;
        if (wanted || G::W256 == 64) {
            v += dpp_mov<kDppRowBcast15, 0xA>(0u, v);
            v += dpp_mov<kDppRowBcast31, 0xC>(0u, v);
            if (lane == 63) {
                if (wanted) atomicAdd(&ksum[k], v);
                if (G::W256 == 64 && wave == 0 && k <= 12) atomicAdd(&ksum256[k], v);
            }
        }
        if (G::W256 == 16 && wave == 0 && lane == 15 && k <= 12) atomicAdd(&ksum256[k], row);
    }
}

__device__ __forceinline__ uint32_t static_k_candidates(uint64_t S, uint32_t n, int lane) {
    const uint32_t k = (uint32_t)lane & 15u;
    const uint64_t fixed = (uint64_t)n * (1u + k);
    const uint64_t upper = (S >> k) + fixed;
    const uint64_t slack = (uint64_t)n * ((1u << k) - 1u);
    const uint64_t lower = (S > slack ? ((S - slack + ((1u << k) - 1u)) >> k) : 0ull) + fixed;
    const uint64_t umin = wave_last_u64(wave_scan_min_u64(lane < 16 ? upper : ~0ull));
    return (uint32_t)__ballot(lane < 16 && lower <= umin) & 0xFFFFu;
}

__device__ __forceinline__ void wave_exclusive_scan_u32(uint32_t* arr, int len, int lane) {
    uint32_t carry = 0;
    for (int base = 0; base < len; base += 64) {
        const int i = base + lane;
        const uint32_t v = (i < len) ? arr[i] : 0u;
        const uint32_t inc = wave_scan_add_u32(v);
        if (i < len) arr[i] = carry + inc - v;
        carry += wave_last_u32(inc);
    }
}

struct SlotGeom {
    int64_t start;
    uint32_t n;
    bool defined;
};

__device__ __forceinline__ uint32_t block_frames(const AnalyzeParams& prm, uint32_t blk) {
    const uint64_t rem = prm.frames - (uint64_t)blk * kMaxBlock;
    return rem < (uint64_t)kMaxBlock ? (uint32_t)rem : (uint32_t)kMaxBlock;
}

__device__ __forceinline__ SlotGeom slot_geom(const AnalyzeParams& prm, uint32_t blk, int slot) {
    SlotGeom g;
    const uint32_t nb = block_frames(prm, blk);
    const int64_t bstart = (int64_t)blk * kMaxBlock;
    const int win = slot >> 2, ch = slot & 3;
    g.defined = true;
    if (prm.channels == 1 && ch != 0) g.defined = false;
    if (win == 0) {
        g.start = bstart;
        g.n = nb;
    } else {
        if (prm.channels != 2 || prm.stereo_mode != 2 || nb <= (uint32_t)kFullCompareLimit) g.defined = false;
        g.n = kProbe;
        g.start = bstart;
        if (g.defined) {
            if (win == 2) g.start = bstart + (nb - kProbe) / 2u;
            if (win == 3) g.start = bstart + nb - kProbe;
        }
    }
    return g;
}

__device__ __forceinline__ StreamDesc wave_uniform(const StreamDesc& d) {
    static_assert(sizeof(StreamDesc) % 4 == 0, "whole words");
    StreamDesc r;
    const uint32_t* src = reinterpret_cast<const uint32_t*>(&d);
    uint32_t* dst = reinterpret_cast<uint32_t*>(&r);
#pragma unroll
    for (size_t i = 0; i < sizeof(StreamDesc) / 4; ++i) dst[i] = (uint32_t)__builtin_amdgcn_readfirstlane((int)src[i]);
    return r;
}

__device__ __forceinline__ StreamDesc stream_of_block(const BatchRef& br, uint32_t gblk) {
    if (br.table == nullptr) return br.single;
    uint32_t lo = 0, hi = br.nstreams;
    while (hi - lo > 1u) {
        const uint32_t mid = (lo + hi) >> 1;
        if (br.table[mid].first_block <= gblk) lo = mid; else hi = mid;
    }
    return br.table[lo];
}
__device__ __forceinline__ StreamDesc stream_of_block_uniform(const BatchRef& br, uint32_t gblk) {
    if (br.table == nullptr) return br.single;
    return wave_uniform(stream_of_block(br, gblk));
}
__device__ __forceinline__ StreamDesc stream_of_workgroup(const BatchRef& br, uint32_t wg) {
    if (br.table == nullptr) return br.single;
    uint32_t lo = 0, hi = br.nstreams;
    while (hi - lo > 1u) {
        const uint32_t mid = (lo + hi) >> 1;
        if (br.table[mid].first_wg <= wg) lo = mid; else hi = mid;
    }
    return wave_uniform(br.table[lo]);
}

__device__ __forceinline__ StreamDesc stream_of_item(const BatchRef& br, uint32_t item) {
    if (br.table == nullptr) return br.single;
    uint32_t lo = 0, hi = br.nstreams;
    while (hi - lo > 1u) {
        const uint32_t mid = (lo + hi) >> 1;
        if (br.table[mid].prm.stream_base <= item) lo = mid; else hi = mid;
    }
    return wave_uniform(br.table[lo]);
}

__device__ __forceinline__ SlotSrc slot_src(const AnalyzeParams& prm, const int32_t* L, const int32_t* R, int ch) {
    SlotSrc s;
    s.kind = ch;
    s.a = L;
    s.b = R;
    s.layout = prm.layout;
    s.channels = prm.channels;
    return s;
}


__device__ __forceinline__ void xcd_slot(uint32_t w, uint32_t per, uint32_t nblocks, uint32_t& blk, uint32_t& which) {
    const uint32_t group = 8u * per, g = w / group, r = w % group;
    if (g < nblocks / 8u) {
        blk = g * 8u + (r & 7u);
        which = r >> 3;
    } else {
        blk = w / per;
        which = w % per;
    }
}

constexpr unsigned long long kRecValid = 1ull << 62, kRecMs = 1ull << 61, kRecFlag = 1ull << 60, kRecBytesMask = (1ull << 60) - 1ull;

__device__ __forceinline__ unsigned long long rec_load(const unsigned long long* p) {
    return __hip_atomic_load(p, __ATOMIC_RELAXED, __HIP_MEMORY_SCOPE_AGENT);
}
__device__ __forceinline__ void rec_store(unsigned long long* p, unsigned long long v) {
    __hip_atomic_store(p, v, __ATOMIC_RELAXED, __HIP_MEMORY_SCOPE_AGENT);
}


__device__ __forceinline__ void lds_barrier() {
    asm volatile("s_waitcnt lgkmcnt(0)\n\ts_barrier" ::: "memory");
}

}
```

### lossless-audio-codec_amd/csrc/k_analyze.hip

```cpp
#include <hip/hip_runtime.h>

#include <cstdlib>
#include <mutex>

#include "emit_device.h"
#include "kernels_internal.h"

namespace lacx {

#ifdef LACX_STAMPS
__device__ unsigned long long g_stamp_acc[40];
#endif

#ifdef LACX_TEST_HOOKS
#define LACX_HOOK(prm, bits) (((prm).debug_skip & (bits)) != 0u)
#else
#define LACX_HOOK(prm, bits) false
#endif

struct PendingSlot {
    long long idx;
    uint32_t done, silent;
};

template <class G>
__device__ __forceinline__ void fused_emit(Smem<G>& sh, Thread<G>& th, const AnalyzeParams& prm, const FuseArgs& fa,
                                           const long long idx, const bool flag_byte, const uint32_t flag_value,
                                           const int tid, PendingSlot* defer, const uint32_t tmpl_key,
                                           const uint32_t* plan_stored, const int plan_words STAMP_PARAMS) {
    const uint32_t n = th.n;
    asm volatile("" : "+v"(th.tid), "+v"(th.a));
    const unsigned long long my_size = (unsigned long long)sh.plan.payload_bytes + (flag_byte ? 1u : 0u);
    if (tid == 0) rec_store(&fa.size_rec[idx], kRecValid | (flag_value ? kRecMs : 0ull) | (flag_byte ? kRecFlag : 0ull) | my_size);
    const bool skip = (unsigned long long)sh.plan.payload_bytes + 16u > fa.slot_stride ||
                      (LACX_HOOK(prm, 1024u) && (idx % 5 == 3));
    bool done = false;
    if (!skip) {
        emit_load_plan(sh, sh.plan, tid, G::T);
        __syncthreads();
        if (sh.plan_any_zr) {
            emit_first_nonzero(th, sh);
            const int32_t nxinc = scan_nx_part1<G>(sh, tid, sh.wx);
            __syncthreads();
            scan_nx_part2<G>(sh, tid, nxinc, sh.wx, (int32_t)n);
            __syncthreads();
        }
        uint8_t* slot = fa.slots + (unsigned long long)idx * fa.slot_stride;
        STAMP(24);
        done = emit_body<G>(sh, th, n, slot, fa.err_flag, [slot](uint8_t** o) { *o = slot; return true; }, tid,
                            LACX_HOOK(prm, 2048u), (uint32_t)fa.slot_stride STAMP_ARGS);
    }
    if (tmpl_key != 0u && done && sh.payload_bytes <= kSilentBytes) {
        SilentTemplate* t = fa.silent;
        if (tid == 0) sh.tmpl_state = atomicCAS(&t->state, 0u, 1u);
        __syncthreads();
        if (sh.tmpl_state == 0u) {
            const uint32_t nv = (sh.payload_bytes + 15u) >> 4;
            const uint32_t* tw = sh.xp.o.obits;
            for (uint32_t v = tid; v < nv; v += G::T) {
                uint4 o;
                o.x = __builtin_bswap32(tw[4u * v]);
                o.y = __builtin_bswap32(tw[4u * v + 1u]);
                o.z = __builtin_bswap32(tw[4u * v + 2u]);
                o.w = __builtin_bswap32(tw[4u * v + 3u]);
                reinterpret_cast<uint4*>(t->bytes)[v] = o;
            }
            if (tid < plan_words) t->plan[tid] = plan_stored[tid];
            if (tid == 0) {
                t->nbytes = sh.payload_bytes;
                t->plan_words = (uint32_t)plan_words;
            }
            asm volatile("s_waitcnt vmcnt(0)" ::: "memory");
            __syncthreads();
            if (tid == 0) __hip_atomic_store(&t->state, tmpl_key, __ATOMIC_RELEASE, __HIP_MEMORY_SCOPE_AGENT);
        }
    }
    if (defer) {
        if (tid == 0) {
            defer->idx = idx;
            defer->done = done ? 1u : 0u;
            defer->silent = LACX_HOOK(prm, 8192u) ? 1u : 0u;
        }
        return;
    }
    asm volatile("s_waitcnt vmcnt(0)" ::: "memory");
    __syncthreads();
    if (tid == 0) {
        if (done) fa.emitted[idx] = 2u;
        if (!LACX_HOOK(prm, 8192u)) rec_store(&fa.ready_rec[idx], done ? 1ull : 2ull);
    }
}

__device__ __forceinline__ void publish_pending(const FuseArgs& fa, PendingSlot& pend, int tid) {
    if (tid == 0) {
        const long long idx = pend.idx;
        if (idx >= 0) {
            if (pend.done) fa.emitted[idx] = 2u;
            if (!pend.silent) rec_store(&fa.ready_rec[idx], pend.done ? 1ull : 2ull);
        }
        pend.idx = -1;
    }
}

template <class G>
__device__ __forceinline__ void score_candidate_wave(Smem<G>& sh, int cand, uint32_t n, int zero_run, uint32_t k0,
                                                     const uint32_t* planeTot, const unsigned long long* acc, int lane,
                                                     bool ksums, uint32_t kmask) {
    uint64_t key = ~0ull;
    if (ksums) {
        if (lane < 16 && ((kmask >> lane) & 1u)) key = (((uint64_t)planeTot[lane] + (uint64_t)n * (uint64_t)(1 + lane)) << 4) | (uint64_t)lane;
    } else {
        const int b = 29 - lane;
        const uint64_t w = (lane < 30) ? ((uint64_t)planeTot[b] << b) : 0ull;
        const uint64_t tk = wave_scan_add_u64(w);
        if (lane >= 14 && lane < 30 && ((kmask >> b) & 1u)) key = (((tk >> b) + (uint64_t)n * (uint64_t)(1 + b)) << 4) | (uint64_t)b;
    }
    const uint64_t best_key = wave_last_u64(wave_scan_min_u64(key));
    if (lane == 0) {
        const uint64_t sbits = best_key >> 4;
        const uint32_t sk = (uint32_t)(best_key & 15u);
        const uint64_t rice = acc[0], bin = acc[1];
        const uint32_t hasrun = acc[3] != 0;
        const uint64_t zr = (zero_run && hasrun) ? acc[2] : rice;
        const uint64_t a = rice < sbits ? rice : sbits;
        const uint64_t c = zr < bin ? zr : bin;
        const uint64_t best = a < c ? a : c;
        if (sh.best_cand < 0 || best < sh.best_bits || (best == sh.best_bits && cand < sh.best_cand)) {
            sh.best_cand = cand;
            sh.best_bits = best;
            sh.best_rice = rice;
            sh.best_zr = zr;
            sh.best_bin = bin;
            sh.best_static = sbits;
            sh.best_k0 = k0;
            sh.best_sk = sk;
            sh.best_hasrun = hasrun;
        }
    }
}

__device__ __forceinline__ uint32_t initial_k_wave(const uint32_t* planes256, uint32_t n, int lane, bool ksums) {
    const uint32_t m = n < 256u ? n : 256u;
    uint64_t key = ~0ull;
    if (ksums) {
        if (lane <= 12) key = (((uint64_t)planes256[lane] + (uint64_t)m * (uint64_t)(1 + lane)) << 4) | (uint64_t)lane;
    } else {
        const int b = 29 - lane;
        const uint64_t w = (lane < 30) ? ((uint64_t)planes256[b] << b) : 0ull;
        const uint64_t tk = wave_scan_add_u64(w);
        if (lane >= 17 && lane < 30) key = (((tk >> b) + (uint64_t)m * (uint64_t)(1 + b)) << 4) | (uint64_t)b;
    }
    return (uint32_t)(wave_last_u64(wave_scan_min_u64(key)) & 15u);
}

template <class G>
__device__ __forceinline__ void slot_sync() {
    if constexpr (G::T == 64) {
        asm volatile("s_waitcnt lgkmcnt(0)" ::: "memory");
    } else {
        __syncthreads();
    }
}

template <class G>
__device__ __forceinline__ void analyze_slot(unsigned char* smem_raw, const AnalyzeParams& prm, uint32_t n_in,
                                             const SlotSrc& src, int64_t start, const LpcSet* __restrict__ lpc_slot,
                                             ChannelPlan* __restrict__ plan_out, int tid, const FuseArgs& fuse,
                                             const long long fuse_idx, const bool fuse_flag_byte,
                                             const uint32_t fuse_flag_value, PendingSlot* pend) {
    Smem<G>& sh = *reinterpret_cast<Smem<G>*>(smem_raw);
    const uint32_t n = n_in;
#ifdef LACX_STAMPS
    unsigned long long stamp_acc[40];
    for (int k = 0; k < 40; ++k) stamp_acc[k] = 0;
    unsigned long long stamp_prev = __builtin_amdgcn_s_memtime();
    const unsigned long long stamp_rt0 = __builtin_amdgcn_s_memrealtime();
#endif
    Thread<G> th;
    thread_init(th, n, tid);
    const uint32_t chunk_bits = stage_samples(th, sh, src, start);
    {
        const bool wave_silent = __ballot(chunk_bits != 0u) == 0ull;
        if ((tid & 63) == 0) sh.wtotF[tid >> 6] = wave_silent ? 0u : 1u;
    }
    for (int i = tid; i < (int)(sizeof(LpcSet) / 2); i += G::T)
        reinterpret_cast<uint16_t*>(&sh.lpc)[i] = reinterpret_cast<const uint16_t*>(lpc_slot)[i];
    if (tid < 32) {
        sh.planeTot[0][tid] = sh.planeTot[1][tid] = 0;
        sh.planeTot256[0][tid] = sh.planeTot256[1][tid] = 0;
    }
    if (tid < 4) sh.acc[0][tid] = sh.acc[1][tid] = 0;
    if (tid < 33) (&sh.lbacc[0][0])[tid] = 0;
    if (tid < 2) sh.has4[tid] = 0;
    if (tid == 0) {
        sh.best_cand = -1;
        sh.tabUZ[G::T] = sh.tabUZ[G::T + 1] = 0;
    }
    if (pend) asm volatile("s_waitcnt vmcnt(0)" ::: "memory");
    slot_sync<G>();
    if (pend) publish_pending(fuse, *pend, tid);
    STAMP(0);

    auto run_pass1 = [&](const bool real) {
        asm volatile("" : "+v"(th.a));
        const bool lpc_off = LACX_HOOK(prm, 16u);
        const uint32_t per_thread = 34u * (uint32_t)G::CH;
        const int32_t left = (int32_t)n - (int32_t)((tid >> 6) * 64 * G::CH);
        const uint32_t valid = left <= 0 ? 0u : (left >= 64 * G::CH ? (uint32_t)(64 * G::CH) : (uint32_t)left);
        const uint32_t beyond = (uint32_t)(64 * G::CH) - valid;
        auto reduce_pair = [&](int c0, const BoundPartials& b0, bool two, const BoundPartials& b1) {
            const uint32_t lo = per_thread - b0.msum, hi = two ? per_thread - b1.msum : 0u;
            const uint32_t g2 = wave_sum_u32(lo | (hi << 16));
            const uint32_t cnt0 = wave_sum_u32(bound_counts<G::CH>(b0));
            const uint32_t cnt1 = two ? wave_sum_u32(bound_counts<G::CH>(b1)) : 0u;
            if ((tid & 63) == 0 && real) {
#pragma unroll
                for (int h = 0; h < 2; ++h) {
                    if (h == 0 || two) {
                        const uint32_t g = h ? (g2 >> 16) : (g2 & 0xFFFFu);
                        const uint32_t cnt = h ? cnt1 : cnt0;
                        const uint32_t nz = cnt & 0x7FFu, n4 = (cnt >> 11) & 0x7FFu, ends = cnt >> 22;
                        atomicAdd(&sh.lbacc[c0 + h][0], g - nz - beyond);
                        atomicAdd(&sh.lbacc[c0 + h][1], (nz - beyond) + (n4 << 16));
                        atomicAdd(&sh.lbacc[c0 + h][2], ends);
                    }
                }
            }
        };
        {
            BoundPartials bf[6];
            if (n == (uint32_t)G::MAXN) pass1_bounds_fixed<G, true>(th, sh, bf);
            else pass1_bounds_fixed<G, false>(th, sh, bf);
#pragma unroll
            for (int c = 0; c < 6; c += 2) reduce_pair(c, bf[c], true, bf[c + 1]);
        }
        asm volatile("" : "+v"(th.a));
        {
            BoundPartials bl[5];
            if (n == (uint32_t)G::MAXN) pass1_bounds_lpc<G, true>(th, sh, lpc_off, bl);
            else pass1_bounds_lpc<G, false>(th, sh, lpc_off, bl);
            reduce_pair(6, bl[0], true, bl[1]);
            reduce_pair(8, bl[2], true, bl[3]);
            reduce_pair(10, bl[4], false, bl[4]);
        }
    };
    bool silent = true;
#pragma unroll
    for (int w = 0; w < G::T / 64; ++w) silent = silent && sh.wtotF[w] == 0u;
    uint32_t tmpl_key = 0;
    if (silent) {
        uint32_t key = 0;
        if constexpr (G::T == 1024) {
            if (fuse.silent && !LACX_HOOK(prm, ~0u)) {
                key = 0x80000000u | (prm.zero_run ? 0x40000000u : 0u) | (prm.partitioning ? 0x20000000u : 0u) | n;
                if (tid == 0) sh.tmpl_state = __hip_atomic_load(&fuse.silent->state, __ATOMIC_RELAXED, __HIP_MEMORY_SCOPE_AGENT);
            }
        }
        STAMP(2);
        slot_sync<G>();
        if constexpr (G::T == 1024) {
            if (key) {
                const uint32_t state = (uint32_t)__builtin_amdgcn_readfirstlane((int)sh.tmpl_state);
                if (state == key) {
                    __builtin_amdgcn_fence(__ATOMIC_ACQUIRE, "agent");
                    const SilentTemplate* t = fuse.silent;
                    const uint32_t nbytes = t->nbytes;
                    if (tid == 0 && fuse.silent_copies) atomicAdd(fuse.silent_copies, 1u);
                    if ((uint32_t)tid < t->plan_words) reinterpret_cast<uint32_t*>(plan_out)[tid] = t->plan[tid];
                    if (fuse_idx >= 0) {
                        if (tid == 0)
                            rec_store(&fuse.size_rec[fuse_idx], kRecValid | (fuse_flag_value ? kRecMs : 0ull) | (fuse_flag_byte ? kRecFlag : 0ull) |
                                                                    ((unsigned long long)nbytes + (fuse_flag_byte ? 1u : 0u)));
                        typedef unsigned int u32x4 __attribute__((ext_vector_type(4)));
                        uint8_t* slot = fuse.slots + (unsigned long long)fuse_idx * fuse.slot_stride;
                        const __amdgpu_buffer_rsrc_t rsrc = __builtin_amdgcn_make_buffer_rsrc(slot, 0, (int)fuse.slot_stride, 0x00020000);
                        const uint32_t nv = (nbytes + 15u) >> 4;
                        for (uint32_t v = tid; v < nv; v += G::T) {
                            const uint4 w = reinterpret_cast<const uint4*>(t->bytes)[v];
                            u32x4 o;
                            o.x = w.x;
                            o.y = w.y;
                            o.z = w.z;
                            o.w = w.w;
                            __builtin_amdgcn_raw_buffer_store_b128(o, rsrc, (int)(16u * v), 0, 16 );
                        }
                        if (pend) {
                            if (tid == 0) {
                                pend->idx = fuse_idx;
                                pend->done = 1u;
                                pend->silent = 0u;
                            }
                        } else {
                            asm volatile("s_waitcnt vmcnt(0)" ::: "memory");
                            __syncthreads();
                            if (tid == 0) {
                                fuse.emitted[fuse_idx] = 2u;
                                rec_store(&fuse.ready_rec[fuse_idx], 1ull);
                            }
                        }
                    }
                    return;
                }
                if (state == 0u && fuse_idx >= 0) tmpl_key = key;
            }
        }
        if (tid <= 10) sh.cand_key[tid] = tid == 0 ? 0ull : ~0ull;
    } else {
#if defined(LACX_STAMPS) && LACX_STAMPS == 3
    {
        uint32_t trips = 2;
        asm volatile("" : "+s"(trips));
        for (uint32_t r = 0; r < trips; ++r) {
            run_pass1(r == 0);
            if (r == 0) STAMP(2); else STAMP(15);
        }
    }
#else
    run_pass1(true);
    STAMP(2);
#endif
    slot_sync<G>();
    if (tid <= 10) {
        const bool avail = !((tid >= 6 && (sh.lpc.used[tid >= 6 ? tid - 6 : 0] == 0 || LACX_HOOK(prm, 16u))) ||
                             (tid >= 1 && LACX_HOOK(prm, 64u)));
        sh.cand_key[tid] = avail ? ((candidate_lower_bound(sh.lbacc[tid][0], sh.lbacc[tid][1], sh.lbacc[tid][2], n, prm.zero_run) << 4) | (uint64_t)tid)
                                 : ~0ull;
    }
    }
    STAMP(5);

    int pending = -1;
    uint32_t pending_k0 = 0;
    bool pending_ksums = false;
    uint32_t pending_kmask = 0xFFFFu;
    uint32_t tried = 0;
    int parity = 0;
    for (;;) {
        asm volatile("" : "+v"(tid));
        if (tid < 64) {
            if (pending >= 0) {
                score_candidate_wave(sh, pending, n, prm.zero_run, pending_k0, sh.planeTot[parity ^ 1], sh.acc[parity ^ 1], tid, pending_ksums, pending_kmask);
                if (tid < 32) sh.planeTot[parity ^ 1][tid] = sh.planeTot256[parity ^ 1][tid] = 0;
                if (tid < 4) sh.acc[parity ^ 1][tid] = 0;
            }
            const uint64_t key = (tid <= 10 && !((tried >> tid) & 1u)) ? sh.cand_key[tid] : ~0ull;
            const uint64_t best_key = wave_last_u64(wave_scan_min_u64(key));
            if (tid == 0) {
                sh.has4[parity] = 0;
                sh.bqcount = 0;
                int next = best_key == ~0ull ? -1 : (int)(best_key & 15u);
                if (next >= 0 && !LACX_HOOK(prm, 128u) && candidate_pruned(best_key >> 4, next, sh.best_bits, sh.best_cand)) next = -1;
                sh.next_cand = next;
            }
        }
        STAMP(1);
        slot_sync<G>();
        STAMP(4);
        const int cand = sh.next_cand;
        if (cand < 0) break;
        tried |= 1u << cand;
        asm volatile("" : "+v"(th.a));
        uint32_t* pt = sh.planeTot[parity];
        uint32_t* pt256 = sh.planeTot256[parity];
        unsigned long long* acc = sh.acc[parity];
        {
            uint32_t ures[G::CH];
            phase_r_residual(th, sh, cand, ures);
            phase_r_store(th, sh, ures);
        }
        ScanRegs<G> sr;
        scan_pz_part1(sh, tid, sr);
        STAMP(3);
        slot_sync<G>();
        const uint64_t total_u = scan_pz_part2(sh, tid, sr);
        const bool narrow = total_u < kNarrowLimit;
        const bool ksums = narrow && !LACX_HOOK(prm, 262144u);
        const uint32_t kmask = !LACX_HOOK(prm, 1048576u) ? static_k_candidates(total_u, n, tid & 63) : 0xFFFFu;
        if (!LACX_HOOK(prm, 1u)) {
            if (ksums) ksums_wave(th, pt, pt256, tid, kmask);
            else plane_totals_wave(th, pt, pt256, tid, kmask ? (int)__builtin_ctz(kmask) : 0);
        }
        if (tid < 64) {
            const uint32_t k0w = initial_k_wave(pt256, n, tid, ksums);
            if (tid == 0) sh.cur_k0 = k0w;
        }
        STAMP(6);
        if (LACX_HOOK(prm, 2u)) {
            sh.tabF[tid] = 0;
            th.has4 = 1u;
        } else if (narrow) {
            phase_a<G, true>(th, sh);
        } else {
            phase_a<G, false>(th, sh);
        }
        if (__ballot(th.has4 != 0u) != 0ull && (tid & 63) == 0) sh.has4[parity] = 1u;
        STAMP(8);
        slot_sync<G>();
        STAMP(10);
        const uint32_t k0 = sh.cur_k0;
        asm volatile("" : "+v"(th.tid));
        if (LACX_HOOK(prm, 4u)) {
            th.crice = th.cbin = th.czr = 1;
            th.chasrun = 0;
        } else {
            const bool zr = prm.zero_run && sh.has4[parity] != 0u;
            const bool full = n == (uint32_t)G::MAXN;
            if (G::T == 64 || LACX_HOOK(prm, 524288u)) {
                phase_b_dispatch<G>(th, sh, k0, narrow, zr, full);
                if ((uint32_t)th.a >= n) {
                    th.crice = th.cbin = th.czr = 0;
                    th.chasrun = 0;
                }
            } else {
                const bool live = (uint32_t)th.a < n;
                bool quick = false;
                if (tid >= 64 && live) quick = phase_b_quick_dispatch<G>(th, sh, narrow, zr);
                if (!quick) {
                    th.crice = th.cbin = th.czr = 0;
                    th.chasrun = 0;
                }
                if (tid >= 64) {
                    const unsigned long long slow = __ballot(live && !quick);
                    if (slow != 0ull) {
                        uint32_t base = 0;
                        if ((tid & 63) == 0) base = atomicAdd(&sh.bqcount, (uint32_t)__popcll(slow));
                        base = (uint32_t)__builtin_amdgcn_readfirstlane((int)base);
                        if (live && !quick) sh.bqueue[base + __builtin_amdgcn_mbcnt_hi((uint32_t)(slow >> 32), __builtin_amdgcn_mbcnt_lo((uint32_t)slow, 0u))] = (uint16_t)tid;
                    }
                }
                STAMP(11);
                slot_sync<G>();
                if (tid < 64) {
                    if (live) phase_b_dispatch<G>(th, sh, k0, narrow, zr, full, false);
                } else {
                    const int w = tid >> 6;
                    const int order = (w & 3) ? (w - 1 - (w >> 2)) : (11 + (w >> 2));
                    const uint32_t qn = sh.bqcount;
                    for (uint32_t e0 = (uint32_t)order * 64u; e0 < qn; e0 += 15u * 64u) {
                        const uint32_t e = e0 + (uint32_t)(tid & 63);
                        if (e < qn) phase_b_queued<G>(th, sh, (int)sh.bqueue[e], k0, narrow, zr, full);
                    }
                }
            }
        }
        STAMP(12);
        {
            const uint64_t r0 = wave_sum_u64(th.crice);
            const uint64_t r1 = wave_sum_u64(th.cbin);
            const uint64_t r2 = wave_sum_u64(th.czr);
            const uint32_t r3 = wave_or_u32(th.chasrun);
            if ((tid & 63) == 0) {
                atomicAdd(&acc[0], (unsigned long long)r0);
                atomicAdd(&acc[1], (unsigned long long)r1);
                atomicAdd(&acc[2], (unsigned long long)r2);
                atomicAdd(&acc[3], (unsigned long long)r3);
            }
        }
        STAMP(13);
        slot_sync<G>();
        STAMP(14);
        pending = cand;
        pending_k0 = k0;
        pending_ksums = ksums;
        pending_kmask = kmask;
        parity ^= 1;
    }

    STAMP(15);
    asm volatile("" : "+v"(tid), "+v"(th.tid), "+v"(th.a));
    const int best = sh.best_cand;
    int max_p = 0;
    if (prm.partitioning && n >= (uint32_t)kMinPartition) max_p = max_partition_order(n);
    const int nseg = max_p > 0 ? ((2 << max_p) - 2) : 0;
    PartMem<G>& pm = sh.xp.part;
    auto clear_partition_scratch = [&]() {
        for (int i = tid; i < nseg; i += G::T) {
            pm.segacc[i][0] = pm.segacc[i][1] = pm.segacc[i][2] = 0;
            pm.segrun[i] = 0;
        }
        if (tid <= G::MAXP) pm.pbits[tid] = 0;
    };
    if (best == pending && !LACX_HOOK(prm, 16384u)) {
        clear_partition_scratch();
        slot_sync<G>();
    } else {
        phase_r(th, sh, best);
        ScanRegs<G> sr;
        scan_pz_part1(sh, tid, sr);
        slot_sync<G>();
        clear_partition_scratch();
        scan_pz_part2(sh, tid, sr);
        slot_sync<G>();
    }
    const bool pnarrow = sh.tabP[G::T] < kNarrowLimit;
    STAMP(16);
    if (max_p > 0) {
        {
            constexpr int kLog = G::TPG == 4 ? 2 : 4;
            static_assert(G::TPG == 4 || G::TPG == 16, "lanes per 64-sample group");
            uint32_t words[15];
            packed_planes(th, words);
            const bool last = (tid & (G::TPG - 1)) == G::TPG - 1;
#pragma unroll
            for (int w = 0; w < 15; ++w) {
                const uint32_t v = seg_sum_u32<kLog>(words[w]);
                if (last) pm.grp[w][tid / G::TPG] = v;
            }
            if (tid < 15) pm.grp[tid][G::NG] = 0;
        }
        slot_sync<G>();
        {
            constexpr int NW = G::T / 64;
            const int wave = tid >> 6, lane = tid & 63;
            for (int w = wave; w < 15; w += NW) wave_exclusive_scan_u32(pm.grp[w], G::NG + 1, lane);
        }
        slot_sync<G>();
        STAMP(17);
        for (int idx = tid; idx < (LACX_HOOK(prm, 32u) ? 0 : nseg); idx += G::T) {
            const int p = 31 - __clz(idx + 2);
            seg_static_eval(sh, n, p, (uint32_t)(idx + 2 - (1 << p)));
        }
        slot_sync<G>();
        STAMP(18);
        auto flush = [&pm](uint32_t idx, unsigned long long rc, unsigned long long bn, unsigned long long zr,
                           uint32_t hr) {
            atomicAdd(&pm.segacc[idx][0], rc);
            atomicAdd(&pm.segacc[idx][1], bn);
            atomicAdd(&pm.segacc[idx][2], zr);
            if (hr) atomicOr(&pm.segrun[idx], 1u);
        };
        if (LACX_HOOK(prm, 8u)) {
        } else if (pnarrow && partitions_chunk_aligned<G>(n, max_p)) {
            const bool ablate_flush = LACX_HOOK(prm, 65536u);
            const uint32_t chunks = n / (uint32_t)G::CH;
            const bool pow2 = (chunks & (chunks - 1u)) == 0u && !LACX_HOOK(prm, 131072u);
            auto seg_flush = [&](int q, uint32_t idx, uint32_t rc, uint32_t bn, uint32_t zr, uint32_t hr, bool with_zr) {
                if (ablate_flush) return;
                const uint32_t lanes = chunks >> (q + 1);
                if (pow2 && lanes >= 2u) {
                    const int lg = lanes >= 64u ? 6 : 31 - __clz((int)lanes);
                    const bool last = ((uint32_t)tid & ((1u << lg) - 1u)) == (1u << lg) - 1u;
                    rc = seg_sum_u32(rc, lg);
                    bn = seg_sum_u32(bn, lg);
                    if (with_zr) zr = seg_sum_u32(zr, lg);
                    if (last) {
                        atomicAdd(reinterpret_cast<uint32_t*>(&pm.segacc[idx][0]), rc);
                        atomicAdd(reinterpret_cast<uint32_t*>(&pm.segacc[idx][1]), bn);
                        if (with_zr) atomicAdd(reinterpret_cast<uint32_t*>(&pm.segacc[idx][2]), zr);
                    }
                } else {
                    atomicAdd(reinterpret_cast<uint32_t*>(&pm.segacc[idx][0]), rc);
                    atomicAdd(reinterpret_cast<uint32_t*>(&pm.segacc[idx][1]), bn);
                    if (with_zr) atomicAdd(reinterpret_cast<uint32_t*>(&pm.segacc[idx][2]), zr);
                }
                if (hr) atomicOr(&pm.segrun[idx], 1u);
            };
            auto flush32 = [&](int q, uint32_t idx, uint32_t rc, uint32_t bn, uint32_t zr, uint32_t hr) {
                seg_flush(q, idx, rc, bn, zr, hr, true);
            };
            auto flush32_nozr = [&](int q, uint32_t idx, uint32_t rc, uint32_t bn, uint32_t, uint32_t) {
                seg_flush(q, idx, rc, bn, 0u, 0u, false);
            };
            auto flush_entry = [&pm, ablate_flush](uint32_t idx, uint32_t rc, uint32_t bn, uint32_t zr, uint32_t hr) {
                if (ablate_flush) return;
                atomicAdd(reinterpret_cast<uint32_t*>(&pm.segacc[idx][0]), rc);
                atomicAdd(reinterpret_cast<uint32_t*>(&pm.segacc[idx][1]), bn);
                if (zr) atomicAdd(reinterpret_cast<uint32_t*>(&pm.segacc[idx][2]), zr);
                if (hr) atomicOr(&pm.segrun[idx], 1u);
            };
            const bool with_zr = prm.zero_run && sh.best_hasrun;
            if (LACX_HOOK(prm, 32768u)) {
                if (with_zr) partition_fused<G, true>(th, sh, max_p, flush32);
                else partition_fused<G, false>(th, sh, max_p, flush32_nozr);
            } else {
                uint16_t* wq = &pm.queue[(tid >> 6) * 64 * G::MAXP];
                uint32_t queued = 0;
                auto enqueue = [&](uint32_t entry, bool ambiguous) {
                    const unsigned long long m = __ballot(ambiguous);
                    if (ambiguous) wq[queued + __builtin_amdgcn_mbcnt_hi((uint32_t)(m >> 32), __builtin_amdgcn_mbcnt_lo((uint32_t)m, 0u))] = (uint16_t)entry;
                    queued += (uint32_t)__popcll(m);
                };
                asm volatile("" : "+v"(th.tid));
                if (!with_zr) {
                    partition_quick<G>(th, sh, max_p, flush32_nozr, enqueue);
                } else {
                    QuickPrep<G> qp;
                    partition_quick_prepare<G>(th, sh, max_p, qp);
                    uint32_t pairs = 0;
                    for (int q = 0; q < max_p; ++q) pairs += (uint32_t)__popcll(__ballot((qp.amb >> q) & 1u));
                    if (pairs > kQuickMaxPairs) partition_fused<G, true>(th, sh, max_p, flush32);
                    else partition_quick_costs<G>(th, sh, max_p, qp, flush32, enqueue);
                }
                STAMP(7);
                if constexpr (G::T > 64) {
                    constexpr int NW = G::T / 64;
                    static_assert(NW <= 16, "one count per wave");
                    const int lane = tid & 63;
                    if (lane == 0) pm.wqcount[tid >> 6] = queued;
                    __syncthreads();
                    const uint32_t mine = lane < NW ? pm.wqcount[lane] : 0u;
                    const uint32_t incl = wave_scan_add_u32(mine);
                    const uint32_t total = (uint32_t)__builtin_amdgcn_readlane((int)incl, NW - 1);
                    for (uint32_t e0 = (uint32_t)(tid & ~63); e0 < total; e0 += (uint32_t)G::T) {
                        const bool live = e0 + (uint32_t)lane < total;
                        const uint32_t e = live ? e0 + (uint32_t)lane : total - 1u;
                        uint32_t w = 0;
#pragma unroll
                        for (int step = NW / 2; step >= 1; step >>= 1) {
                            const uint32_t probe = (uint32_t)__shfl((int)incl, (int)(w + (uint32_t)step - 1u), 64);
                            w += probe <= e ? (uint32_t)step : 0u;
                        }
                        const uint32_t prev = (uint32_t)__shfl((int)incl, (int)(w ? w - 1u : 0u), 64);
                        const uint32_t before = w ? prev : 0u;
                        const uint32_t entry = pm.queue[w * 64u * (uint32_t)G::MAXP + (e - before)];
                        if (live) {
                            if (with_zr) partition_slow_entry<G, true>(sh, n, entry, flush_entry);
                            else partition_slow_entry<G, false>(sh, n, entry, flush_entry);
                        }
                    }
                } else {
                    asm volatile("s_waitcnt lgkmcnt(0)" ::: "memory");
                    for (uint32_t e = (uint32_t)(tid & 63); e < queued; e += 64u) {
                        if (with_zr) partition_slow_entry<G, true>(sh, n, wq[e], flush_entry);
                        else partition_slow_entry<G, false>(sh, n, wq[e], flush_entry);
                    }
                }
                STAMP(9);
            }
        } else {
            for (int p = 1; p <= max_p; ++p) {
                if (pnarrow) {
                    partition_pass<G, true>(th, sh, p, flush);
                } else {
                    partition_pass<G, false>(th, sh, p, flush);
                }
            }
        }
        STAMP(19);
        slot_sync<G>();
        STAMP(20);
        for (int j0 = tid & ~63; j0 < nseg + 2; j0 += G::T) {
            const int j = j0 + (tid & 63), idx = j - 2;
            const bool valid = j >= 2 && idx < nseg;
            const unsigned long long bits = valid ? seg_choose(sh, (uint32_t)idx, prm.zero_run) : 0ull;
            if (j0 >= 64) {
                const unsigned long long sum = wave_sum_u64(bits);
                if ((tid & 63) == 0) atomicAdd(&pm.pbits[31 - __clz(j0)], sum);
            } else if (valid) {
                atomicAdd(&pm.pbits[31 - __clz(j)], bits);
            }
        }
        slot_sync<G>();
    }
    if (tid == 0) finalize_plan(sh, n, prm.zero_run, max_p, &sh.plan);
    slot_sync<G>();
    const int plan_words = (int)(offsetof(ChannelPlan, part_mode_k) + ((size_t)1 << sh.plan.partition_order) + 3) / 4;
    for (int i = tid; i < plan_words; i += G::T)
        reinterpret_cast<uint32_t*>(plan_out)[i] = reinterpret_cast<const uint32_t*>(&sh.plan)[i];
    STAMP(21);
    if constexpr (G::T == 1024) {
        if (fuse_idx >= 0) fused_emit<G>(sh, th, prm, fuse, fuse_idx, fuse_flag_byte, fuse_flag_value, tid, pend, tmpl_key,
                                        reinterpret_cast<const uint32_t*>(plan_out), plan_words STAMP_ARGS);
    }
    STAMP(23);
#if defined(LACX_STAMPS) && (LACX_STAMPS == 1 || LACX_STAMPS == 3)
    if ((tid & 63) == 0 && (tid >> 6) == (int)(blockIdx.x & 15u) && G::T == 1024) {
        stamp_acc[22] = __builtin_amdgcn_s_memrealtime() - stamp_rt0;
        for (int k = 0; k < 32; ++k) atomicAdd(&g_stamp_acc[k], stamp_acc[k]);
        atomicAdd(&g_stamp_acc[32], 1ull);
    }
#endif
}

#ifndef LACX_PROBE_WAVES
#define LACX_PROBE_WAVES 6
#endif
#ifndef LACX_PROBE_WG_WAVES
#define LACX_PROBE_WG_WAVES 1
#endif
constexpr int kProbeWaves = LACX_PROBE_WG_WAVES;
template <class G>
struct TailArgs {};
template <>
struct TailArgs<GProbe> {
    uint32_t* front_ctr;
    BlockPlan* bplans;
    uint32_t* need_full_out;
};
template <class G>
__global__ __launch_bounds__(G::T == 64 ? 64 * kProbeWaves : G::T, G::T == 64 ? LACX_PROBE_WAVES : 4) void k_analyze(BatchRef br, int probe_class, uint32_t one_block,
                                                  int which_base, const LpcSet* __restrict__ lpcs,
                                                  const uint32_t* __restrict__ need,
                                                  ChannelPlan* __restrict__ plans,
                                                  unsigned long long* __restrict__ t_first,
                                                  unsigned long long* __restrict__ t_last, FuseArgs fuse,
                                                  uint32_t* __restrict__ work_ctr, uint32_t total_wg, uint32_t pair_blocks,
                                                  TailArgs<G> tail) {
    extern __shared__ __align__(16) unsigned char smem_all[];
    __shared__ uint32_t s_next;
    __shared__ PendingSlot s_pend;
    static_assert(sizeof(Smem<G>) % 16 == 0, "slot images are 16-byte aligned");
    const int tid = G::T == 64 ? (int)(threadIdx.x & 63u) : (int)threadIdx.x;
    unsigned char* smem_raw = smem_all + (G::T == 64 ? (size_t)(threadIdx.x >> 6) * sizeof(Smem<G>) : 0);
    if (t_first && tid == 0) atomicMax(t_first, ~(unsigned long long)__builtin_amdgcn_s_memrealtime());
    const bool persistent = work_ctr != nullptr;
    uint32_t rep = 0;
    uint32_t v = G::T == 64 ? blockIdx.x * (uint32_t)kProbeWaves + (uint32_t)__builtin_amdgcn_readfirstlane((int)(threadIdx.x >> 6)) : blockIdx.x;
    if (persistent) {
        if (tid == 0) {
            s_next = atomicAdd(work_ctr, 1u);
            s_pend.idx = -1;
        }
        __syncthreads();
        v = (uint32_t)__builtin_amdgcn_readfirstlane((int)s_next);
    }
    for (;;) {
        if (persistent && v >= total_wg) break;
        uint32_t blk;
        uint32_t reps = 1u;
        int slot = -1;
        int which_in_block = -1;
        uint32_t needed_slots = 0;
        StreamDesc sd;
        if (probe_class) {
            blk = v / 12u;
            sd = stream_of_block_uniform(br, blk);
            const int s = 4 + (int)(v % 12u);
            if (((uint32_t)__builtin_amdgcn_readfirstlane((int)need[blk]) >> s) & 1u) slot = s;
        } else {
            uint32_t wsel;
            if (which_base) {
                blk = one_block;
                sd = stream_of_block_uniform(br, blk);
                wsel = v;
            } else if (persistent && pair_blocks != 0u) {
                sd = br.single;
                uint32_t lblk;
                if (v < pair_blocks) {
                    lblk = v;
                    wsel = rep;
                    reps = 2u;
                } else {
                    const uint32_t s = v - pair_blocks;
                    lblk = pair_blocks + (s >> 1);
                    wsel = s & 1u;
                }
                blk = sd.first_block + lblk;
            } else {
                sd = stream_of_workgroup(br, v);
                const uint32_t per = sd.prm.channels == 2 ? 2u : 1u;
                uint32_t lblk;
                xcd_slot(v - sd.first_wg, per, LACX_HOOK(sd.prm, 512u) ? 0u : sd.prm.num_blocks, lblk, wsel);
                blk = sd.first_block + lblk;
            }
            int which = (int)wsel + which_base;
            which_in_block = which;
            uint32_t m = (uint32_t)__builtin_amdgcn_readfirstlane((int)need[blk]) & 0xFu;
            needed_slots = (uint32_t)__popc(m);
            while (m) {
                const int s = __ffs((int)m) - 1;
                if (which == 0) {
                    slot = s;
                    break;
                }
                --which;
                m &= m - 1u;
            }
        }
        if (slot >= 0) {
            const AnalyzeParams prm = sd.prm;
            const uint32_t lblk = blk - sd.first_block;
            const SlotGeom g = slot_geom(prm, lblk, slot);
            const uint32_t n = g.n;
            const size_t sidx = (size_t)blk * kSlotsPerBlock + slot;
            const SlotSrc src = slot_src(prm, sd.left, sd.right, slot & 3);

            long long fuse_idx = -1;
            bool flag_byte = false;
            if (fuse.slots && !probe_class && !which_base) {
                const uint32_t item = lblk * (uint32_t)prm.channels + (uint32_t)which_in_block;
                fuse_idx = (long long)prm.stream_base + item;
                flag_byte = prm.channels == 2 && prm.stereo_mode == 2 && which_in_block == 0;
                if (item >= sd.fuse_items || needed_slots != (uint32_t)prm.channels) fuse_idx = -1;
            }
            int slot_tid = tid;
            asm volatile("" : "+v"(slot_tid));
            analyze_slot<G>(smem_raw, prm, n, src, g.start, &lpcs[sidx], &plans[sidx], slot_tid, fuse, fuse_idx, flag_byte,
                            (uint32_t)((slot & 3) >= 2 ? 1u : 0u), persistent ? &s_pend : nullptr);
            if (t_last && tid == 0) atomicMax(t_last, (unsigned long long)__builtin_amdgcn_s_memrealtime());
            if constexpr (G::T == 64) {
                uint32_t* const front_ctr = tail.front_ctr;
                if (probe_class && front_ctr) {
                    uint32_t last = 0;
                    if (tid == 0) {
                        ChannelPlan* po = &plans[sidx];
                        agent_store(&po->payload_bytes, reinterpret_cast<Smem<G>*>(smem_raw)->plan.payload_bytes);
                        asm volatile("s_waitcnt vmcnt(0)" ::: "memory");
                        last = atomicAdd(&front_ctr[(size_t)blk * 2 + 1], 1u) == 11u ? 1u : 0u;
                    }
                    if (__builtin_amdgcn_readfirstlane((int)last)) {
                        if (tid == 0) front_ctr[(size_t)blk * 2 + 1] = 0u;
                        if (tid < 16) decide_probed_block(blk, tid, tail.bplans, tail.need_full_out, plans);
                    }
                }
            }
        }
        if (!persistent) break;
        __syncthreads();
        if (++rep < reps) continue;
        rep = 0;
        if (tid == 0) s_next = atomicAdd(work_ctr, 1u);
        __syncthreads();
        v = (uint32_t)__builtin_amdgcn_readfirstlane((int)s_next);
    }
    if (persistent) {
        asm volatile("s_waitcnt vmcnt(0)" ::: "memory");
        __syncthreads();
        publish_pending(fuse, s_pend, tid);
    }
}

size_t analyze_smem_bytes_full() { return sizeof(Smem<GFull>); }

int debug_read_stamps(unsigned long long* out32) {
#ifdef LACX_STAMPS
    if (hipMemcpyFromSymbol(out32, HIP_SYMBOL(g_stamp_acc), sizeof(unsigned long long) * 40) != hipSuccess) return 0;
    unsigned long long zero[40] = {0};
    (void)hipMemcpyToSymbol(HIP_SYMBOL(g_stamp_acc), zero, sizeof(zero));
    return 1;
#else
    (void)out32;
    return 0;
#endif
}
size_t analyze_smem_bytes_probe() { return sizeof(Smem<GProbe>); }

hipError_t ensure_kernel_attrs() {
    static std::mutex mu;
    static bool done[kMaxDevices] = {};
    int dev = -1;
    hipError_t e = hipGetDevice(&dev);
    if (e != hipSuccess) return e;
    if (dev < 0 || dev >= kMaxDevices) return hipErrorInvalidDevice;
    std::lock_guard<std::mutex> lock(mu);
    if (done[dev]) return hipSuccess;
    e = hipFuncSetAttribute(reinterpret_cast<const void*>(&k_analyze<GFull>),
                            hipFuncAttributeMaxDynamicSharedMemorySize, (int)sizeof(Smem<GFull>));
    if (e == hipSuccess) e = set_kernel_attrs_front();
    if (e == hipSuccess)
        e = hipFuncSetAttribute(reinterpret_cast<const void*>(&k_analyze<GProbe>),
                                hipFuncAttributeMaxDynamicSharedMemorySize, (int)(sizeof(Smem<GProbe>) * kProbeWaves));
    if (e == hipSuccess) e = set_kernel_attrs_emit();
    if (e == hipSuccess) done[dev] = true;
    return e;
}

static uint32_t compute_units() {
    static std::mutex mu;
    static int cus[kMaxDevices] = {};
    int dev = 0;
    if (hipGetDevice(&dev) != hipSuccess || dev < 0 || dev >= kMaxDevices) return 256u;
    std::lock_guard<std::mutex> lock(mu);
    if (cus[dev] == 0) {
        int n = 0;
        cus[dev] = (hipDeviceGetAttribute(&n, hipDeviceAttributeMultiprocessorCount, dev) == hipSuccess && n > 0) ? n : 256;
    }
    return (uint32_t)cus[dev];
}

hipError_t launch_analysis(const LaunchSet& ls, const DeviceWorkspace& ws, hipStream_t stream, hipEvent_t* ev,
                           const FuseArgs* fuse, hipEvent_t wait_before_full, const LaunchTuning& tune) {
    const FuseArgs fa = fuse ? *fuse : FuseArgs{};
    hipError_t e = ensure_kernel_attrs();
    if (e != hipSuccess) return e;
    const BatchRef& br = ls.br;
    const uint32_t nb = br.total_blocks;
    if (nb == 0) return hipSuccess;
    hipStream_t full_stream = stream;
    if (tune.front_stream && ev) stream = tune.front_stream;
    if (ev) (void)hipEventRecord(ev[0], stream);
    e = hipMemsetAsync(ws.plans, 0, sizeof(ChannelPlan) * (size_t)nb * kSlotsPerBlock, stream);
    if (e != hipSuccess) return e;
    bool any_auto = false, any_both = false;
    uint32_t total_wg = 0;
    for (uint32_t i = 0; i < ls.nstreams; ++i) {
        const AnalyzeParams& p = ls.streams[i].prm;
        const bool autost = p.channels == 2 && p.stereo_mode == 2;
        any_auto = any_auto || autost;
        any_both = any_both || (autost && p.frames - (uint64_t)(p.num_blocks - 1) * kMaxBlock <= (uint64_t)kFullCompareLimit);
        total_wg += p.num_blocks * (p.channels == 2 ? 2u : 1u);
    }
    auto launch_front = [&](const BatchRef& r, const DeviceWorkspace& w, uint32_t cnt, hipStream_t st, bool mark) {
        uint32_t* fc = tune.fold_front ? w.front_ctr : nullptr;
        hipLaunchKernelGGL(k_ingest, dim3(cnt * 4u), dim3(kIngestThreads), 0, st, r, w.sums, w.badidx, w.acorr, fc, w.bplans,
                           w.need_probe, w.need_full);
        if (!fc) hipLaunchKernelGGL(k_stereo, dim3((cnt + 3) / 4), dim3(64), 0, st, r, w.sums, w.badidx, w.bplans, w.need_probe, w.need_full);
        hipLaunchKernelGGL(k_levinson, dim3((cnt * kSlotsPerBlock + kLevThreads - 1) / kLevThreads), dim3(kLevThreads),
                           sizeof(LevMem), st, r, w.acorr, w.need_probe, w.lpcs);
        if (mark && ev) (void)hipEventRecord(ev[1], st);
        if (any_auto) {
            static_assert(12 % kProbeWaves == 0, "whole workgroups per block");
            hipLaunchKernelGGL(k_analyze<GProbe>, dim3(cnt * (12u / kProbeWaves)), dim3(GProbe::T * kProbeWaves), sizeof(Smem<GProbe>) * kProbeWaves, st, r, 1, 0u, 0,
                               w.lpcs, w.need_probe, w.plans, (unsigned long long*)nullptr, (unsigned long long*)nullptr, FuseArgs{},
                               (uint32_t*)nullptr, 0u, 0u, TailArgs<GProbe>{fc, w.bplans, w.need_full});
            if (!fc) hipLaunchKernelGGL(k_decide, dim3((cnt + 3) / 4), dim3(64), 0, st, r, 1, w.bplans, w.need_probe, w.need_full, w.plans);
        }
    };
    const bool halves = tune.aux_stream && tune.aux_ev[0] && tune.aux_ev[1] && br.table == nullptr && ls.nstreams == 1 && nb >= 1024u;
    if (halves) {
        const AnalyzeParams& p = br.single.prm;
        const uint32_t nb1 = (nb / 2u) & ~7u;
        const uint64_t frame_bytes = p.layout == PCM_INTERLEAVED_I16 ? 2ull * (uint64_t)p.channels
                                                                     : (p.layout == PCM_INTERLEAVED_I24 ? 3ull * (uint64_t)p.channels : 4ull);
        auto sub = [&](uint32_t b0, uint32_t cnt) {
            BatchRef r = br;
            StreamDesc& sd = r.single;
            const uint64_t f0 = (uint64_t)b0 * kMaxBlock;
            const uint64_t f1 = p.frames < (uint64_t)(b0 + cnt) * kMaxBlock ? p.frames : (uint64_t)(b0 + cnt) * kMaxBlock;
            sd.prm.frames = f1 - f0;
            sd.prm.num_blocks = cnt;
            r.total_blocks = cnt;
            sd.left = reinterpret_cast<const int32_t*>(reinterpret_cast<const uint8_t*>(br.single.left) + f0 * frame_bytes);
            sd.right = (p.layout == PCM_PLANAR_I32 && br.single.right) ? br.single.right + f0 : nullptr;
            return r;
        };
        auto wsub = [&](uint32_t b0) {
            DeviceWorkspace w = ws;
            const size_t sl = (size_t)b0 * kSlotsPerBlock;
            w.plans += sl;
            w.bplans += b0;
            w.need_probe += b0;
            w.need_full += b0;
            w.acorr += sl * 13;
            w.lpcs += sl;
            w.sums += (size_t)b0 * 12;
            w.badidx += (size_t)b0 * 2;
            if (w.front_ctr) w.front_ctr += (size_t)b0 * 2;
            return w;
        };
        hipError_t he = hipEventRecord(tune.aux_ev[0], stream);
        if (he == hipSuccess) he = hipStreamWaitEvent(tune.aux_stream, tune.aux_ev[0], 0);
        if (he != hipSuccess) return he;
        launch_front(sub(0, nb1), ws, nb1, stream, true);
        launch_front(sub(nb1, nb - nb1), wsub(nb1), nb - nb1, tune.aux_stream, false);
        he = hipEventRecord(tune.aux_ev[1], tune.aux_stream);
        if (he == hipSuccess) he = hipStreamWaitEvent(stream, tune.aux_ev[1], 0);
        if (he != hipSuccess) return he;
    } else {
        launch_front(br, ws, nb, stream, true);
    }
    if (ev) (void)hipEventRecord(ev[2], stream);
    if (full_stream != stream) {
        const hipError_t we = hipStreamWaitEvent(full_stream, ev[2], 0);
        if (we != hipSuccess) return we;
        stream = full_stream;
    }
    if (wait_before_full) {
        const hipError_t we = hipStreamWaitEvent(stream, wait_before_full, 0);
        if (we != hipSuccess) return we;
    }
    const bool persistent = analysis_is_persistent(ws);
    const uint32_t pgrid = tune.persistent_grid ? tune.persistent_grid : compute_units();
    uint32_t pair_blocks = 0, units = total_wg;
    if (persistent && !tune.no_pairs && br.table == nullptr && ls.nstreams == 1 && ls.streams[0].prm.channels == 2 && nb > pgrid) {
        pair_blocks = nb - pgrid;
        units = pair_blocks + 2u * (nb - pair_blocks);
    }
    const uint32_t grid = persistent ? (units < pgrid ? units : pgrid) : total_wg;
    hipLaunchKernelGGL(k_analyze<GFull>, dim3(grid), dim3(GFull::T), sizeof(Smem<GFull>), stream, br, 0, 0u, 0,
                       ws.lpcs, ws.need_full, ws.plans, ws.t_first, ws.t_last, fa, persistent ? ws.work_ctr : (uint32_t*)nullptr,
                       units, pair_blocks, TailArgs<GFull>{});
    if (any_both) {
        for (uint32_t i = 0; i < ls.nstreams; ++i) {
            const StreamDesc& sd = ls.streams[i];
            const AnalyzeParams& p = sd.prm;
            if (p.channels == 2 && p.stereo_mode == 2 && p.frames - (uint64_t)(p.num_blocks - 1) * kMaxBlock <= (uint64_t)kFullCompareLimit)
                hipLaunchKernelGGL(k_analyze<GFull>, dim3(2), dim3(GFull::T), sizeof(Smem<GFull>), stream, br, 0,
                                   sd.first_block + p.num_blocks - 1u, 2, ws.lpcs, ws.need_full, ws.plans,
                                   (unsigned long long*)nullptr, (unsigned long long*)nullptr, FuseArgs{}, (uint32_t*)nullptr, 0u, 0u,
                                   TailArgs<GFull>{});
        }
    }
    if (ev) (void)hipEventRecord(ev[3], stream);
    if (any_both) {
        hipLaunchKernelGGL(k_decide, dim3((nb + 3) / 4), dim3(64), 0, stream, br, 2, ws.bplans, ws.need_probe,
                           ws.need_full, ws.plans);
    }
    if (ev) (void)hipEventRecord(ev[4], stream);
    return hipGetLastError();
}

}
```

### lossless-audio-codec_amd/csrc/kernels_internal.h

```cpp
#pragma once
#include "device_util.h"
#include "emit_core.h"

namespace lacx {

using GFull = Geo<16, 1024>;
using GProbe = Geo<4, 64>;
constexpr int kMaxDevices = 64;

constexpr int kIngestThreads = 256;
constexpr int kLevThreads = 256;
struct LevMem {
    uint64_t m[3][13][kLevThreads];
    uint32_t es[3][13][kLevThreads];
};
__global__ void k_ingest(BatchRef br, unsigned long long* __restrict__ sums, uint32_t* __restrict__ badidx,
                         int64_t* __restrict__ acorr, uint32_t* __restrict__ front_ctr, BlockPlan* __restrict__ bplans,
                         uint32_t* __restrict__ need_probe, uint32_t* __restrict__ need_full);
__global__ void k_stereo(BatchRef br, const unsigned long long* __restrict__ sums, const uint32_t* __restrict__ badidx,
                         BlockPlan* __restrict__ bplans, uint32_t* __restrict__ need_probe, uint32_t* __restrict__ need_full);
__global__ void k_levinson(BatchRef br, const int64_t* __restrict__ acorr, const uint32_t* __restrict__ need_probe,
                           LpcSet* __restrict__ lpcs);
__global__ void k_decide(BatchRef br, int phase, BlockPlan* __restrict__ bplans, const uint32_t* __restrict__ need_probe,
                         uint32_t* __restrict__ need_full, const ChannelPlan* __restrict__ plans);
hipError_t set_kernel_attrs_front();

template <class T>
__device__ __forceinline__ void agent_store(T* p, T v) { __hip_atomic_store(p, v, __ATOMIC_RELAXED, __HIP_MEMORY_SCOPE_AGENT); }
template <class T>
__device__ __forceinline__ T agent_load(const T* p) { return __hip_atomic_load(p, __ATOMIC_RELAXED, __HIP_MEMORY_SCOPE_AGENT); }

__device__ __forceinline__ void decide_probed_block(uint32_t blk, int sub, BlockPlan* __restrict__ bplans,
                                                    uint32_t* __restrict__ need_full, const ChannelPlan* __restrict__ plans) {
    const uint32_t bytes = sub >= 4 ? agent_load(&plans[(size_t)blk * kSlotsPerBlock + sub].payload_bytes) : 0u;
    const bool is_ms = (sub & 3) >= 2;
    uint32_t lr = is_ms ? 0u : bytes, ms = is_ms ? bytes : 0u;
#pragma unroll
    for (int d = 1; d < 16; d <<= 1) {
        lr += (uint32_t)__shfl_xor((int)lr, d, 64);
        ms += (uint32_t)__shfl_xor((int)ms, d, 64);
    }
    if (sub != 0) return;
    const uint8_t choose_ms = ms < lr;
    bplans[blk].choose_ms = choose_ms;
    need_full[blk] = choose_ms ? 0xCu : 0x3u;
}

hipError_t set_kernel_attrs_emit();

hipError_t ensure_kernel_attrs();

}
```

Measured before the change: 24180.

## Run probe analysis as two 32-lane half-wave slots per wavefront

Changes the probe geometry from 4-sample chunks over 64 threads to 8-sample chunks over 32 threads, so each wavefront analyses two probe slots at once, one per half. It adds half-wave scan, reduce, ballot and rank primitives, an 8-wide adder tree for bit-plane counts, and generalises the scans, slot indexing, shared-memory sizing and launch grid to the slot width. The aim is to halve the number of waves per probe block and cut per-slot wave overhead. In exchange each thread carries more per-thread work, the occupancy target drops from 6 to 4 waves, and the half-wave selects add some instruction overhead.

After: 24950, median of 6. 1.03x the previous value.

```diff
diff --git a/lossless-audio-codec_amd/csrc/analyze_core.h b/lossless-audio-codec_amd/csrc/analyze_core.h
--- a/lossless-audio-codec_amd/csrc/analyze_core.h
+++ b/lossless-audio-codec_amd/csrc/analyze_core.h
@@ -18,6 +18,8 @@
     static constexpr int W96 = 96 / CH_;
     static constexpr int MAXP = (MAXN >= 8192) ? 8 : ((MAXN >= 4096) ? 7 : ((MAXN >= 2048) ? 6 : ((MAXN >= 1024) ? 5 : ((MAXN >= 512) ? 4 : 3))));
     static constexpr int NSEG = (2 << MAXP) - 2;
+    static constexpr int SW = (T_ < 64) ? T_ : 64;
+    static constexpr int NW = (T_ + 63) / 64;
     static_assert(32 % CH_ == 0, "chunk must divide the 96/256 windows");
     static_assert(MAXN % 64 == 0, "whole groups");
 };
@@ -390,7 +392,17 @@
         sliced_add<4>(l3[0], l3[1], l4);
 #pragma unroll
         for (int l = 0; l < G::LV; ++l) cs[l] = l4[l];
+    } else if (G::CH == 8) {
+        uint32_t l1[4][2], l2[2][3], l3[4];
+#pragma unroll
+        for (int i = 0; i < 4; ++i) sliced_add<1>(&u[2 * i], &u[2 * i + 1], l1[i]);
+#pragma unroll
+        for (int i = 0; i < 2; ++i) sliced_add<2>(l1[2 * i], l1[2 * i + 1], l2[i]);
+        sliced_add<3>(l2[0], l2[1], l3);
+#pragma unroll
+        for (int l = 0; l < G::LV; ++l) cs[l] = l3[l];
     } else {
+        static_assert(G::CH == 16 || G::CH == 8 || G::CH == 4, "one adder tree per chunk length");
         uint32_t l1[2][2], l2[3];
         sliced_add<1>(&u[0], &u[1], l1[0]);
         sliced_add<1>(&u[2], &u[3], l1[1]);
diff --git a/lossless-audio-codec_amd/csrc/device_util.h b/lossless-audio-codec_amd/csrc/device_util.h
--- a/lossless-audio-codec_amd/csrc/device_util.h
+++ b/lossless-audio-codec_amd/csrc/device_util.h
@@ -97,6 +97,105 @@
 __device__ __forceinline__ uint32_t wave_sum_u32(uint32_t v) { return wave_last_u32(wave_scan_add_u32(v)); }
 __device__ __forceinline__ uint32_t wave_or_u32(uint32_t v) { return wave_last_u32(wave_scan_or_u32(v)); }
 
+__device__ __forceinline__ bool upper_half() { return (threadIdx.x & 32u) != 0u; }
+
+__device__ __forceinline__ uint32_t half_last_u32(uint32_t v) {
+    const uint32_t lo = (uint32_t)__builtin_amdgcn_readlane((int)v, 31), hi = (uint32_t)__builtin_amdgcn_readlane((int)v, 63);
+    return upper_half() ? hi : lo;
+}
+__device__ __forceinline__ uint64_t half_last_u64(uint64_t v) {
+    return ((uint64_t)half_last_u32((uint32_t)(v >> 32)) << 32) | half_last_u32((uint32_t)v);
+}
+__device__ __forceinline__ uint32_t half_scan_add_u32(uint32_t v) {
+    v += dpp_mov<kDppRowShr1, 0xF>(0u, v);
+    v += dpp_mov<kDppRowShr2, 0xF>(0u, v);
+    v += dpp_mov<kDppRowShr4, 0xF>(0u, v);
+    v += dpp_mov<kDppRowShr8, 0xF>(0u, v);
+    v += dpp_mov<kDppRowBcast15, 0xA>(0u, v);
+    return v;
+}
+__device__ __forceinline__ uint64_t half_scan_add_u64(uint64_t v) {
+    v += dpp_mov64<kDppRowShr1, 0xF>(v);
+    v += dpp_mov64<kDppRowShr2, 0xF>(v);
+    v += dpp_mov64<kDppRowShr4, 0xF>(v);
+    v += dpp_mov64<kDppRowShr8, 0xF>(v);
+    v += dpp_mov64<kDppRowBcast15, 0xA>(v);
+    return v;
+}
+__device__ __forceinline__ int32_t half_scan_max_i32(int32_t v) {
+    constexpr uint32_t kMin = 0x80000000u;
+    auto mx = [](int32_t a, uint32_t b) { return a > (int32_t)b ? a : (int32_t)b; };
+    v = mx(v, dpp_mov<kDppRowShr1, 0xF>(kMin, (uint32_t)v));
+    v = mx(v, dpp_mov<kDppRowShr2, 0xF>(kMin, (uint32_t)v));
+    v = mx(v, dpp_mov<kDppRowShr4, 0xF>(kMin, (uint32_t)v));
+    v = mx(v, dpp_mov<kDppRowShr8, 0xF>(kMin, (uint32_t)v));
+    v = mx(v, dpp_mov<kDppRowBcast15, 0xA>(kMin, (uint32_t)v));
+    return v;
+}
+__device__ __forceinline__ uint32_t half_scan_or_u32(uint32_t v) {
+    v |= dpp_mov<kDppRowShr1, 0xF>(0u, v);
+    v |= dpp_mov<kDppRowShr2, 0xF>(0u, v);
+    v |= dpp_mov<kDppRowShr4, 0xF>(0u, v);
+    v |= dpp_mov<kDppRowShr8, 0xF>(0u, v);
+    v |= dpp_mov<kDppRowBcast15, 0xA>(0u, v);
+    return v;
+}
+__device__ __forceinline__ uint64_t half_scan_min_u64(uint64_t v) {
+    auto step = [](uint64_t a, uint32_t lo, uint32_t hi) {
+        const uint64_t b = ((uint64_t)hi << 32) | lo;
+        return b < a ? b : a;
+    };
+#define LACX_MIN_STEP(CTRL, MASK) \
+    v = step(v, dpp_mov<CTRL, MASK>(0xFFFFFFFFu, (uint32_t)v), dpp_mov<CTRL, MASK>(0xFFFFFFFFu, (uint32_t)(v >> 32)))
+    LACX_MIN_STEP(kDppRowShr1, 0xF);
+    LACX_MIN_STEP(kDppRowShr2, 0xF);
+    LACX_MIN_STEP(kDppRowShr4, 0xF);
+    LACX_MIN_STEP(kDppRowShr8, 0xF);
+    LACX_MIN_STEP(kDppRowBcast15, 0xA);
+#undef LACX_MIN_STEP
+    return v;
+}
+__device__ __forceinline__ uint64_t half_sum_u64(uint64_t v) { return half_last_u64(half_scan_add_u64(v)); }
+__device__ __forceinline__ uint32_t half_sum_u32(uint32_t v) { return half_last_u32(half_scan_add_u32(v)); }
+__device__ __forceinline__ uint32_t half_or_u32(uint32_t v) { return half_last_u32(half_scan_or_u32(v)); }
+template <int SW> constexpr auto slot_last_u32 = SW == 64 ? &wave_last_u32 : &half_last_u32;
+template <int SW> constexpr auto slot_last_u64 = SW == 64 ? &wave_last_u64 : &half_last_u64;
+template <int SW> constexpr auto slot_scan_add_u32 = SW == 64 ? &wave_scan_add_u32 : &half_scan_add_u32;
+template <int SW> constexpr auto slot_scan_add_u64 = SW == 64 ? &wave_scan_add_u64 : &half_scan_add_u64;
+template <int SW> constexpr auto slot_scan_max_i32 = SW == 64 ? &wave_scan_max_i32 : &half_scan_max_i32;
+template <int SW> constexpr auto slot_scan_or_u32 = SW == 64 ? &wave_scan_or_u32 : &half_scan_or_u32;
+template <int SW> constexpr auto slot_scan_min_u64 = SW == 64 ? &wave_scan_min_u64 : &half_scan_min_u64;
+template <int SW> constexpr auto slot_sum_u64 = SW == 64 ? &wave_sum_u64 : &half_sum_u64;
+template <int SW> constexpr auto slot_sum_u32 = SW == 64 ? &wave_sum_u32 : &half_sum_u32;
+template <int SW> constexpr auto slot_or_u32 = SW == 64 ? &wave_or_u32 : &half_or_u32;
+template <int SW>
+__device__ __forceinline__ uint32_t slot_first_u32(uint32_t v) {
+    static_assert(SW == 64 || SW == 32, "the wave or one of its halves");
+    if constexpr (SW == 64) {
+        return (uint32_t)__builtin_amdgcn_readfirstlane((int)v);
+    } else {
+        const uint32_t lo = (uint32_t)__builtin_amdgcn_readlane((int)v, 0), hi = (uint32_t)__builtin_amdgcn_readlane((int)v, 32);
+        return upper_half() ? hi : lo;
+    }
+}
+template <int SW>
+__device__ __forceinline__ uint64_t slot_ballot(bool pred) {
+    const unsigned long long m = __ballot(pred);
+    if constexpr (SW == 64) {
+        return m;
+    } else {
+        return upper_half() ? (uint32_t)(m >> 32) : (uint32_t)m;
+    }
+}
+template <int SW>
+__device__ __forceinline__ uint32_t slot_rank(uint64_t m) {
+    if constexpr (SW == 64) {
+        return __builtin_amdgcn_mbcnt_hi((uint32_t)(m >> 32), __builtin_amdgcn_mbcnt_lo((uint32_t)m, 0u));
+    } else {
+        return (uint32_t)__popc((uint32_t)m & ((1u << (threadIdx.x & 31u)) - 1u));
+    }
+}
+
 template <int LOG>
 __device__ __forceinline__ uint32_t seg_sum_u32(uint32_t v) {
     if (LOG >= 1) v += dpp_mov<kDppRowShr1, 0xF>(0u, v);
@@ -129,11 +228,11 @@
     const int lane = tid & 63, wave = tid >> 6;
     r.v = sh.tabP[tid];
     r.z = sh.tabNZ[tid];
-    const uint64_t inc = wave_scan_add_u64(r.v);
-    const int32_t zinc = wave_scan_max_i32(r.z);
+    const uint64_t inc = slot_scan_add_u64<G::SW>(r.v);
+    const int32_t zinc = slot_scan_max_i32<G::SW>(r.z);
     r.inc = inc;
     r.zinc = zinc;
-    if (lane == 63) {
+    if (lane == G::SW - 1) {
         sh.wtotP[wave] = inc;
         sh.wtotZ[wave] = zinc;
     }
@@ -145,7 +244,7 @@
     uint64_t base = 0, total = 0;
     int32_t zbase = -1;
 #pragma unroll
-    for (int w = 0; w < G::T / 64; ++w) {
+    for (int w = 0; w < G::NW; ++w) {
         const uint64_t pw = sh.wtotP[w];
         const int32_t z = sh.wtotZ[w];
         total += pw;
@@ -154,7 +253,7 @@
             zbase = z > zbase ? z : zbase;
         }
     }
-    int32_t zprev = __shfl_up(r.zinc, 1, 64);
+    int32_t zprev = __shfl_up(r.zinc, 1, G::SW);
     if (lane == 0) zprev = -1;
     sh.tabP[tid] = base + r.inc - r.v;
     sh.tabNZ[tid] = zprev > zbase ? zprev : zbase;
@@ -172,6 +271,22 @@
     uint32_t any = 0;
 #pragma unroll
     for (int l = 0; l < G::LV; ++l) any |= th.cs[l];
+    if constexpr (G::SW == 32) {
+        const int nplanes = 32 - __clz((int)slot_or_u32<32>(any));
+        uint32_t mine = 0;
+        for (int b = 0; b < nplanes; ++b) {
+            uint32_t tot = 0;
+#pragma unroll
+            for (int l = 0; l < G::LV; ++l) tot += (uint32_t)__popc((uint32_t)slot_ballot<32>((th.cs[l] >> b) & 1u)) << l;
+            if (lane == b) mine = tot;
+        }
+        static_assert(G::SW != 32 || G::W256 == G::SW, "the slot is its own first 256 samples");
+        if (lane < nplanes) {
+            if (lane >= first_plane) atomicAdd(&planeTot[lane], mine);
+            atomicAdd(&planeTot256[lane], mine);
+        }
+        return;
+    }
     const int nplanes = 32 - __clz((int)wave_or_u32(any));
     const uint64_t m256 = (G::W256 >= 64) ? ~0ull : ((1ull << (G::W256 & 63)) - 1ull);
     uint32_t mine = 0, mine256 = 0;
@@ -198,7 +313,7 @@
 template <class G>
 __device__ __forceinline__ void ksums_wave(const Thread<G>& th, uint32_t* ksum, uint32_t* ksum256, int tid, uint32_t kmask = 0xFFFFu) {
     const int lane = tid & 63, wave = tid >> 6;
-    static_assert(G::W256 == 16 || G::W256 == 64, "the first 256 samples are one DPP row or the whole wave");
+    static_assert(G::W256 == 16 || G::W256 == G::SW, "the first 256 samples are one DPP row or the slot's whole share of the wave");
 #pragma unroll
     for (int k = 0; k < 16; ++k) {
         const bool wanted = ((kmask >> k) & 1u) != 0u;
@@ -212,36 +327,38 @@
         v += dpp_mov<kDppRowShr4, 0xF>(0u, v);
         v += dpp_mov<kDppRowShr8, 0xF>(0u, v);
         const uint32_t row = v;
-        if (wanted || G::W256 == 64) {
+        if (wanted || G::W256 == G::SW) {
             v += dpp_mov<kDppRowBcast15, 0xA>(0u, v);
-            v += dpp_mov<kDppRowBcast31, 0xC>(0u, v);
-            if (lane == 63) {
+            if constexpr (G::SW == 64) v += dpp_mov<kDppRowBcast31, 0xC>(0u, v);
+            if (lane == G::SW - 1) {
                 if (wanted) atomicAdd(&ksum[k], v);
-                if (G::W256 == 64 && wave == 0 && k <= 12) atomicAdd(&ksum256[k], v);
+                if (G::W256 == G::SW && wave == 0 && k <= 12) atomicAdd(&ksum256[k], v);
             }
         }
         if (G::W256 == 16 && wave == 0 && lane == 15 && k <= 12) atomicAdd(&ksum256[k], row);
     }
 }
 
+template <int SW = 64>
 __device__ __forceinline__ uint32_t static_k_candidates(uint64_t S, uint32_t n, int lane) {
     const uint32_t k = (uint32_t)lane & 15u;
     const uint64_t fixed = (uint64_t)n * (1u + k);
     const uint64_t upper = (S >> k) + fixed;
     const uint64_t slack = (uint64_t)n * ((1u << k) - 1u);
     const uint64_t lower = (S > slack ? ((S - slack + ((1u << k) - 1u)) >> k) : 0ull) + fixed;
-    const uint64_t umin = wave_last_u64(wave_scan_min_u64(lane < 16 ? upper : ~0ull));
-    return (uint32_t)__ballot(lane < 16 && lower <= umin) & 0xFFFFu;
-}
-
+    const uint64_t umin = slot_last_u64<SW>(slot_scan_min_u64<SW>(lane < 16 ? upper : ~0ull));
+    return (uint32_t)slot_ballot<SW>(lane < 16 && lower <= umin) & 0xFFFFu;
+}
+
+template <int SW = 64>
 __device__ __forceinline__ void wave_exclusive_scan_u32(uint32_t* arr, int len, int lane) {
     uint32_t carry = 0;
-    for (int base = 0; base < len; base += 64) {
+    for (int base = 0; base < len; base += SW) {
         const int i = base + lane;
         const uint32_t v = (i < len) ? arr[i] : 0u;
-        const uint32_t inc = wave_scan_add_u32(v);
+        const uint32_t inc = slot_scan_add_u32<SW>(v);
         if (i < len) arr[i] = carry + inc - v;
-        carry += wave_last_u32(inc);
+        carry += slot_last_u32<SW>(inc);
     }
 }
 
diff --git a/lossless-audio-codec_amd/csrc/k_analyze.hip b/lossless-audio-codec_amd/csrc/k_analyze.hip
--- a/lossless-audio-codec_amd/csrc/k_analyze.hip
+++ b/lossless-audio-codec_amd/csrc/k_analyze.hip
@@ -112,10 +112,10 @@
     } else {
         const int b = 29 - lane;
         const uint64_t w = (lane < 30) ? ((uint64_t)planeTot[b] << b) : 0ull;
-        const uint64_t tk = wave_scan_add_u64(w);
+        const uint64_t tk = slot_scan_add_u64<G::SW>(w);
         if (lane >= 14 && lane < 30 && ((kmask >> b) & 1u)) key = (((tk >> b) + (uint64_t)n * (uint64_t)(1 + b)) << 4) | (uint64_t)b;
     }
-    const uint64_t best_key = wave_last_u64(wave_scan_min_u64(key));
+    const uint64_t best_key = slot_last_u64<G::SW>(slot_scan_min_u64<G::SW>(key));
     if (lane == 0) {
         const uint64_t sbits = best_key >> 4;
         const uint32_t sk = (uint32_t)(best_key & 15u);
@@ -139,6 +139,7 @@
     }
 }
 
+template <int SW>
 __device__ __forceinline__ uint32_t initial_k_wave(const uint32_t* planes256, uint32_t n, int lane, bool ksums) {
     const uint32_t m = n < 256u ? n : 256u;
     uint64_t key = ~0ull;
@@ -147,15 +148,15 @@
     } else {
         const int b = 29 - lane;
         const uint64_t w = (lane < 30) ? ((uint64_t)planes256[b] << b) : 0ull;
-        const uint64_t tk = wave_scan_add_u64(w);
+        const uint64_t tk = slot_scan_add_u64<SW>(w);
         if (lane >= 17 && lane < 30) key = (((tk >> b) + (uint64_t)m * (uint64_t)(1 + b)) << 4) | (uint64_t)b;
     }
-    return (uint32_t)(wave_last_u64(wave_scan_min_u64(key)) & 15u);
+    return (uint32_t)(slot_last_u64<SW>(slot_scan_min_u64<SW>(key)) & 15u);
 }
 
 template <class G>
 __device__ __forceinline__ void slot_sync() {
-    if constexpr (G::T == 64) {
+    if constexpr (G::T <= 64) {
         asm volatile("s_waitcnt lgkmcnt(0)" ::: "memory");
     } else {
         __syncthreads();
@@ -180,7 +181,7 @@
     thread_init(th, n, tid);
     const uint32_t chunk_bits = stage_samples(th, sh, src, start);
     {
-        const bool wave_silent = __ballot(chunk_bits != 0u) == 0ull;
+        const bool wave_silent = slot_ballot<G::SW>(chunk_bits != 0u) == 0ull;
         if ((tid & 63) == 0) sh.wtotF[tid >> 6] = wave_silent ? 0u : 1u;
     }
     for (int i = tid; i < (int)(sizeof(LpcSet) / 2); i += G::T)
@@ -190,7 +191,11 @@
         sh.planeTot256[0][tid] = sh.planeTot256[1][tid] = 0;
     }
     if (tid < 4) sh.acc[0][tid] = sh.acc[1][tid] = 0;
-    if (tid < 33) (&sh.lbacc[0][0])[tid] = 0;
+    if constexpr (G::T >= 33) {
+        if (tid < 33) (&sh.lbacc[0][0])[tid] = 0;
+    } else {
+        for (int i = tid; i < 33; i += G::T) (&sh.lbacc[0][0])[i] = 0;
+    }
     if (tid < 2) sh.has4[tid] = 0;
     if (tid == 0) {
         sh.best_cand = -1;
@@ -206,13 +211,13 @@
         const bool lpc_off = LACX_HOOK(prm, 16u);
         const uint32_t per_thread = 34u * (uint32_t)G::CH;
         const int32_t left = (int32_t)n - (int32_t)((tid >> 6) * 64 * G::CH);
-        const uint32_t valid = left <= 0 ? 0u : (left >= 64 * G::CH ? (uint32_t)(64 * G::CH) : (uint32_t)left);
-        const uint32_t beyond = (uint32_t)(64 * G::CH) - valid;
+        const uint32_t valid = left <= 0 ? 0u : (left >= G::SW * G::CH ? (uint32_t)(G::SW * G::CH) : (uint32_t)left);
+        const uint32_t beyond = (uint32_t)(G::SW * G::CH) - valid;
         auto reduce_pair = [&](int c0, const BoundPartials& b0, bool two, const BoundPartials& b1) {
             const uint32_t lo = per_thread - b0.msum, hi = two ? per_thread - b1.msum : 0u;
-            const uint32_t g2 = wave_sum_u32(lo | (hi << 16));
-            const uint32_t cnt0 = wave_sum_u32(bound_counts<G::CH>(b0));
-            const uint32_t cnt1 = two ? wave_sum_u32(bound_counts<G::CH>(b1)) : 0u;
+            const uint32_t g2 = slot_sum_u32<G::SW>(lo | (hi << 16));
+            const uint32_t cnt0 = slot_sum_u32<G::SW>(bound_counts<G::CH>(b0));
+            const uint32_t cnt1 = two ? slot_sum_u32<G::SW>(bound_counts<G::CH>(b1)) : 0u;
             if ((tid & 63) == 0 && real) {
 #pragma unroll
                 for (int h = 0; h < 2; ++h) {
@@ -246,7 +251,7 @@
     };
     bool silent = true;
 #pragma unroll
-    for (int w = 0; w < G::T / 64; ++w) silent = silent && sh.wtotF[w] == 0u;
+    for (int w = 0; w < G::NW; ++w) silent = silent && sh.wtotF[w] == 0u;
     uint32_t tmpl_key = 0;
     if (silent) {
         uint32_t key = 0;
@@ -344,7 +349,7 @@
                 if (tid < 4) sh.acc[parity ^ 1][tid] = 0;
             }
             const uint64_t key = (tid <= 10 && !((tried >> tid) & 1u)) ? sh.cand_key[tid] : ~0ull;
-            const uint64_t best_key = wave_last_u64(wave_scan_min_u64(key));
+            const uint64_t best_key = slot_last_u64<G::SW>(slot_scan_min_u64<G::SW>(key));
             if (tid == 0) {
                 sh.has4[parity] = 0;
                 sh.bqcount = 0;
@@ -375,13 +380,13 @@
         const uint64_t total_u = scan_pz_part2(sh, tid, sr);
         const bool narrow = total_u < kNarrowLimit;
         const bool ksums = narrow && !LACX_HOOK(prm, 262144u);
-        const uint32_t kmask = !LACX_HOOK(prm, 1048576u) ? static_k_candidates(total_u, n, tid & 63) : 0xFFFFu;
+        const uint32_t kmask = !LACX_HOOK(prm, 1048576u) ? static_k_candidates<G::SW>(total_u, n, tid & 63) : 0xFFFFu;
         if (!LACX_HOOK(prm, 1u)) {
             if (ksums) ksums_wave(th, pt, pt256, tid, kmask);
             else plane_totals_wave(th, pt, pt256, tid, kmask ? (int)__builtin_ctz(kmask) : 0);
         }
         if (tid < 64) {
-            const uint32_t k0w = initial_k_wave(pt256, n, tid, ksums);
+            const uint32_t k0w = initial_k_wave<G::SW>(pt256, n, tid, ksums);
             if (tid == 0) sh.cur_k0 = k0w;
         }
         STAMP(6);
@@ -393,7 +398,7 @@
         } else {
             phase_a<G, false>(th, sh);
         }
-        if (__ballot(th.has4 != 0u) != 0ull && (tid & 63) == 0) sh.has4[parity] = 1u;
+        if (slot_ballot<G::SW>(th.has4 != 0u) != 0ull && (tid & 63) == 0) sh.has4[parity] = 1u;
         STAMP(8);
         slot_sync<G>();
         STAMP(10);
@@ -405,7 +410,7 @@
         } else {
             const bool zr = prm.zero_run && sh.has4[parity] != 0u;
             const bool full = n == (uint32_t)G::MAXN;
-            if (G::T == 64 || LACX_HOOK(prm, 524288u)) {
+            if (G::T <= 64 || LACX_HOOK(prm, 524288u)) {
                 phase_b_dispatch<G>(th, sh, k0, narrow, zr, full);
                 if ((uint32_t)th.a >= n) {
                     th.crice = th.cbin = th.czr = 0;
@@ -445,10 +450,10 @@
         }
         STAMP(12);
         {
-            const uint64_t r0 = wave_sum_u64(th.crice);
-            const uint64_t r1 = wave_sum_u64(th.cbin);
-            const uint64_t r2 = wave_sum_u64(th.czr);
-            const uint32_t r3 = wave_or_u32(th.chasrun);
+            const uint64_t r0 = slot_sum_u64<G::SW>(th.crice);
+            const uint64_t r1 = slot_sum_u64<G::SW>(th.cbin);
+            const uint64_t r2 = slot_sum_u64<G::SW>(th.czr);
+            const uint32_t r3 = slot_or_u32<G::SW>(th.chasrun);
             if ((tid & 63) == 0) {
                 atomicAdd(&acc[0], (unsigned long long)r0);
                 atomicAdd(&acc[1], (unsigned long long)r1);
@@ -496,8 +501,8 @@
     STAMP(16);
     if (max_p > 0) {
         {
-            constexpr int kLog = G::TPG == 4 ? 2 : 4;
-            static_assert(G::TPG == 4 || G::TPG == 16, "lanes per 64-sample group");
+            constexpr int kLog = G::TPG == 4 ? 2 : (G::TPG == 8 ? 3 : 4);
+            static_assert(G::TPG == 4 || G::TPG == 8 || G::TPG == 16, "lanes per 64-sample group");
             uint32_t words[15];
             packed_planes(th, words);
             const bool last = (tid & (G::TPG - 1)) == G::TPG - 1;
@@ -510,9 +515,9 @@
         }
         slot_sync<G>();
         {
-            constexpr int NW = G::T / 64;
+            constexpr int NW = G::NW;
             const int wave = tid >> 6, lane = tid & 63;
-            for (int w = wave; w < 15; w += NW) wave_exclusive_scan_u32(pm.grp[w], G::NG + 1, lane);
+            for (int w = wave; w < 15; w += NW) wave_exclusive_scan_u32<G::SW>(pm.grp[w], G::NG + 1, lane);
         }
         slot_sync<G>();
         STAMP(17);
@@ -576,8 +581,8 @@
                 uint16_t* wq = &pm.queue[(tid >> 6) * 64 * G::MAXP];
                 uint32_t queued = 0;
                 auto enqueue = [&](uint32_t entry, bool ambiguous) {
-                    const unsigned long long m = __ballot(ambiguous);
-                    if (ambiguous) wq[queued + __builtin_amdgcn_mbcnt_hi((uint32_t)(m >> 32), __builtin_amdgcn_mbcnt_lo((uint32_t)m, 0u))] = (uint16_t)entry;
+                    const unsigned long long m = slot_ballot<G::SW>(ambiguous);
+                    if (ambiguous) wq[queued + slot_rank<G::SW>(m)] = (uint16_t)entry;
                     queued += (uint32_t)__popcll(m);
                 };
                 asm volatile("" : "+v"(th.tid));
@@ -587,7 +592,7 @@
                     QuickPrep<G> qp;
                     partition_quick_prepare<G>(th, sh, max_p, qp);
                     uint32_t pairs = 0;
-                    for (int q = 0; q < max_p; ++q) pairs += (uint32_t)__popcll(__ballot((qp.amb >> q) & 1u));
+                    for (int q = 0; q < max_p; ++q) pairs += (uint32_t)__popcll(slot_ballot<G::SW>((qp.amb >> q) & 1u));
                     if (pairs > kQuickMaxPairs) partition_fused<G, true>(th, sh, max_p, flush32);
                     else partition_quick_costs<G>(th, sh, max_p, qp, flush32, enqueue);
                 }
@@ -620,7 +625,7 @@
                     }
                 } else {
                     asm volatile("s_waitcnt lgkmcnt(0)" ::: "memory");
-                    for (uint32_t e = (uint32_t)(tid & 63); e < queued; e += 64u) {
+                    for (uint32_t e = (uint32_t)(tid & 63); e < queued; e += (uint32_t)G::SW) {
                         if (with_zr) partition_slow_entry<G, true>(sh, n, wq[e], flush_entry);
                         else partition_slow_entry<G, false>(sh, n, wq[e], flush_entry);
                     }
@@ -644,7 +649,7 @@
             const bool valid = j >= 2 && idx < nseg;
             const unsigned long long bits = valid ? seg_choose(sh, (uint32_t)idx, prm.zero_run) : 0ull;
             if (j0 >= 64) {
-                const unsigned long long sum = wave_sum_u64(bits);
+                const unsigned long long sum = slot_sum_u64<G::SW>(bits);
                 if ((tid & 63) == 0) atomicAdd(&pm.pbits[31 - __clz(j0)], sum);
             } else if (valid) {
                 atomicAdd(&pm.pbits[31 - __clz(j)], bits);
@@ -673,12 +678,14 @@
 }
 
 #ifndef LACX_PROBE_WAVES
-#define LACX_PROBE_WAVES 6
+#define LACX_PROBE_WAVES (LACX_PROBE_HALVES ? 4 : 6)
 #endif
 #ifndef LACX_PROBE_WG_WAVES
 #define LACX_PROBE_WG_WAVES 1
 #endif
 constexpr int kProbeWaves = LACX_PROBE_WG_WAVES;
+constexpr int kProbeSlotsPerWave = 64 / GProbe::SW;
+constexpr int kProbeSlotsPerWg = kProbeWaves * kProbeSlotsPerWave;
 template <class G>
 struct TailArgs {};
 template <>
@@ -688,7 +695,7 @@
     uint32_t* need_full_out;
 };
 template <class G>
-__global__ __launch_bounds__(G::T == 64 ? 64 * kProbeWaves : G::T, G::T == 64 ? LACX_PROBE_WAVES : 4) void k_analyze(BatchRef br, int probe_class, uint32_t one_block,
+__global__ __launch_bounds__(G::T <= 64 ? 64 * kProbeWaves : G::T, G::T <= 64 ? LACX_PROBE_WAVES : 4) void k_analyze(BatchRef br, int probe_class, uint32_t one_block,
                                                   int which_base, const LpcSet* __restrict__ lpcs,
                                                   const uint32_t* __restrict__ need,
                                                   ChannelPlan* __restrict__ plans,
@@ -700,12 +707,12 @@
     __shared__ uint32_t s_next;
     __shared__ PendingSlot s_pend;
     static_assert(sizeof(Smem<G>) % 16 == 0, "slot images are 16-byte aligned");
-    const int tid = G::T == 64 ? (int)(threadIdx.x & 63u) : (int)threadIdx.x;
-    unsigned char* smem_raw = smem_all + (G::T == 64 ? (size_t)(threadIdx.x >> 6) * sizeof(Smem<G>) : 0);
+    const int tid = G::T <= 64 ? (int)(threadIdx.x & (uint32_t)(G::SW - 1)) : (int)threadIdx.x;
+    unsigned char* smem_raw = smem_all + (G::T <= 64 ? (size_t)(threadIdx.x / (uint32_t)G::SW) * sizeof(Smem<G>) : 0);
     if (t_first && tid == 0) atomicMax(t_first, ~(unsigned long long)__builtin_amdgcn_s_memrealtime());
     const bool persistent = work_ctr != nullptr;
     uint32_t rep = 0;
-    uint32_t v = G::T == 64 ? blockIdx.x * (uint32_t)kProbeWaves + (uint32_t)__builtin_amdgcn_readfirstlane((int)(threadIdx.x >> 6)) : blockIdx.x;
+    uint32_t v = G::T <= 64 ? blockIdx.x * (uint32_t)kProbeWaves + (uint32_t)__builtin_amdgcn_readfirstlane((int)(threadIdx.x >> 6)) : blockIdx.x;
     if (persistent) {
         if (tid == 0) {
             s_next = atomicAdd(work_ctr, 1u);
@@ -722,10 +729,12 @@
         int which_in_block = -1;
         uint32_t needed_slots = 0;
         StreamDesc sd;
-        if (probe_class) {
-            blk = v / 12u;
+        if (G::SW == 32 || probe_class) {
+            constexpr uint32_t kWavesPerBlock = 12u / (uint32_t)(64 / G::SW);
+            blk = v / kWavesPerBlock;
             sd = stream_of_block_uniform(br, blk);
-            const int s = 4 + (int)(v % 12u);
+            int s = 4 + (int)(v % kWavesPerBlock) * (64 / G::SW);
+            if (G::SW == 32 && upper_half()) s += 1;
             if (((uint32_t)__builtin_amdgcn_readfirstlane((int)need[blk]) >> s) & 1u) slot = s;
         } else {
             uint32_t wsel;
@@ -770,7 +779,7 @@
         if (slot >= 0) {
             const AnalyzeParams prm = sd.prm;
             const uint32_t lblk = blk - sd.first_block;
-            const SlotGeom g = slot_geom(prm, lblk, slot);
+            const SlotGeom g = slot_geom(prm, lblk, G::SW == 32 ? __builtin_amdgcn_readfirstlane(slot & ~1) : slot);
             const uint32_t n = g.n;
             const size_t sidx = (size_t)blk * kSlotsPerBlock + slot;
             const SlotSrc src = slot_src(prm, sd.left, sd.right, slot & 3);
@@ -788,7 +797,7 @@
             analyze_slot<G>(smem_raw, prm, n, src, g.start, &lpcs[sidx], &plans[sidx], slot_tid, fuse, fuse_idx, flag_byte,
                             (uint32_t)((slot & 3) >= 2 ? 1u : 0u), persistent ? &s_pend : nullptr);
             if (t_last && tid == 0) atomicMax(t_last, (unsigned long long)__builtin_amdgcn_s_memrealtime());
-            if constexpr (G::T == 64) {
+            if constexpr (G::T <= 64) {
                 uint32_t* const front_ctr = tail.front_ctr;
                 if (probe_class && front_ctr) {
                     uint32_t last = 0;
@@ -798,7 +807,7 @@
                         asm volatile("s_waitcnt vmcnt(0)" ::: "memory");
                         last = atomicAdd(&front_ctr[(size_t)blk * 2 + 1], 1u) == 11u ? 1u : 0u;
                     }
-                    if (__builtin_amdgcn_readfirstlane((int)last)) {
+                    if (slot_first_u32<G::SW>(last)) {
                         if (tid == 0) front_ctr[(size_t)blk * 2 + 1] = 0u;
                         if (tid < 16) decide_probed_block(blk, tid, tail.bplans, tail.need_full_out, plans);
                     }
@@ -833,7 +842,7 @@
     return 0;
 #endif
 }
-size_t analyze_smem_bytes_probe() { return sizeof(Smem<GProbe>); }
+size_t analyze_smem_bytes_probe() { return sizeof(Smem<GProbe>) * kProbeSlotsPerWave; }
 
 hipError_t ensure_kernel_attrs() {
     static std::mutex mu;
@@ -849,7 +858,7 @@
     if (e == hipSuccess) e = set_kernel_attrs_front();
     if (e == hipSuccess)
         e = hipFuncSetAttribute(reinterpret_cast<const void*>(&k_analyze<GProbe>),
-                                hipFuncAttributeMaxDynamicSharedMemorySize, (int)(sizeof(Smem<GProbe>) * kProbeWaves));
+                                hipFuncAttributeMaxDynamicSharedMemorySize, (int)(sizeof(Smem<GProbe>) * kProbeSlotsPerWg));
     if (e == hipSuccess) e = set_kernel_attrs_emit();
     if (e == hipSuccess) done[dev] = true;
     return e;
@@ -899,8 +908,8 @@
                            sizeof(LevMem), st, r, w.acorr, w.need_probe, w.lpcs);
         if (mark && ev) (void)hipEventRecord(ev[1], st);
         if (any_auto) {
-            static_assert(12 % kProbeWaves == 0, "whole workgroups per block");
-            hipLaunchKernelGGL(k_analyze<GProbe>, dim3(cnt * (12u / kProbeWaves)), dim3(GProbe::T * kProbeWaves), sizeof(Smem<GProbe>) * kProbeWaves, st, r, 1, 0u, 0,
+            static_assert(12 % kProbeSlotsPerWg == 0, "whole workgroups per block");
+            hipLaunchKernelGGL(k_analyze<GProbe>, dim3(cnt * (12u / kProbeSlotsPerWg)), dim3(64 * kProbeWaves), sizeof(Smem<GProbe>) * kProbeSlotsPerWg, st, r, 1, 0u, 0,
                                w.lpcs, w.need_probe, w.plans, (unsigned long long*)nullptr, (unsigned long long*)nullptr, FuseArgs{},
                                (uint32_t*)nullptr, 0u, 0u, TailArgs<GProbe>{fc, w.bplans, w.need_full});
             if (!fc) hipLaunchKernelGGL(k_decide, dim3((cnt + 3) / 4), dim3(64), 0, st, r, 1, w.bplans, w.need_probe, w.need_full, w.plans);
diff --git a/lossless-audio-codec_amd/csrc/kernels_internal.h b/lossless-audio-codec_amd/csrc/kernels_internal.h
--- a/lossless-audio-codec_amd/csrc/kernels_internal.h
+++ b/lossless-audio-codec_amd/csrc/kernels_internal.h
@@ -5,7 +5,14 @@
 namespace lacx {
 
 using GFull = Geo<16, 1024>;
+#ifndef LACX_PROBE_HALVES
+#define LACX_PROBE_HALVES 1
+#endif
+#if LACX_PROBE_HALVES
+using GProbe = Geo<8, 32>;
+#else
 using GProbe = Geo<4, 64>;
+#endif
 constexpr int kMaxDevices = 64;
 
 constexpr int kIngestThreads = 256;
```
